# irfanfadhullah/unet_zoo

Measured on AMD Instinct MI355X. Metric: images/sec (fwd+bwd) at B=16 3x256x256, 1/2/4/8 MI355X, higher is better.
Workload: dtype bf16; 1 GPU; unet train step (zero_grad+fwd+BCE+bwd+clip+AdamW), B=16/GPU 3x256x256, random-init weights; global_batch=16, parallelism=dp1

## Files before the change

### include/unetzoo_hip.h

```cpp
#ifndef UNETZOO_HIP_H
#define UNETZOO_HIP_H

#include <stddef.h>
#include <stdint.h>

#ifdef __cplusplus
extern "C" {
#endif

#define UZ_ABI_VERSION 1

enum { UZ_F32 = 0, UZ_BF16 = 1 };

enum {
  UZ_OK = 0,
  UZ_EINVAL = -1,
  UZ_ENOTIMPL = -2
};

enum {
  UZ_TAPS_CONV = 0,
  UZ_TAPS_GATHER2X2 = 1,
  UZ_TAPS_CONV_UP2 = 2,
  UZ_TAPS_CONV_S2 = 3
// ... 4 lines not shown
};

int uz_abi_version(void);
const char* uz_last_error_string(void);
int uz_profile_arm(void* start_event, void* stop_event);
int uz_profile_disarm(void);
int uz_build_ablate(void);
const char* uz_source_hash(void);
int uz_clock_probe(int iters, void* out_pairs, int workgroups, void* stream);
int uz_set_cu_reserve(int n);
int uz_get_cu_reserve(void);

typedef struct uz_conv_desc {
  int dtype;
  int N, H, W;
  int Hin, Win;
  int Cin, ldx;
  int Nout, ldy;
  int ntaps, taps_mode, dil;
  int store_mode, Co;
  int Hout, Wout;
} uz_conv_desc;

int uz_conv_igemm_grid_m(const uz_conv_desc* d);
int uz_conv_igemm_kernel_name(const uz_conv_desc* d, int with_workspace, char* buf, int cap);
int uz_conv_igemm(const uz_conv_desc* d, const void* x, const void* w_packed, const float* bias,
                  void* y, float* stats_partial, void* stream);
int uz_conv_igemm_res(const uz_conv_desc* d, const void* x, const void* w_packed, const float* bias,
                      const void* res, int ldres, void* y, void* stream);
int uz_conv_igemm_res_ws(const uz_conv_desc* d, const void* x, const void* w_packed, const float* bias,
                         const void* res, int ldres, void* y, void* workspace, void* stream);
long long uz_conv_igemm_workspace_bytes(const uz_conv_desc* d);
int uz_conv_igemm_ws_grid_m(const uz_conv_desc* d);
int uz_conv_igemm_ws(const uz_conv_desc* d, const void* x, const void* w_packed, const float* bias,
                     void* y, float* stats_partial, void* workspace, void* stream);
int uz_conv_igemm_bnred_supported(const uz_conv_desc* d);
int uz_conv_igemm_bnred(const uz_conv_desc* d, const void* x, const void* w_packed, void* y, const void* bn_y,
                        int ld_bny, const float* scale, const float* shift, const float* mean, const float* invstd,
                        float* partial, void* stream);

int uz_conv_igemm_xf_supported(const uz_conv_desc* d);
int uz_conv_igemm_xf(const uz_conv_desc* d, const void* x, const float* in_scale, const float* in_shift,
                     const void* w_packed, const float* bias, void* y, float* stats_partial, void* stream);

int uz_conv_igemm_bnact_supported(const uz_conv_desc* d);
int uz_conv_igemm_bnact(const uz_conv_desc* d, const void* x, const void* w_packed, const float* bias,
                        const float* out_scale, const float* out_shift, int relu, void* y, void* stream);

typedef struct uz_wgrad_desc {
  int dtype;
  int N, H, W;
  int Hr, Wr;
  int Ci, ldl;
  int Cj, ldr;
  int ntaps, taps_mode, dil;
} uz_wgrad_desc;

int uz_wgrad_split(const uz_wgrad_desc* d);
long long uz_wgrad_workspace_bytes(const uz_wgrad_desc* d);
int uz_wgrad(const uz_wgrad_desc* d, const void* L, const void* R, float* out, void* workspace,
             void* stream);
int uz_wgrad_kernel_name(const uz_wgrad_desc* d, char* buf, int cap);
int uz_wgrad_xf_supported(const uz_wgrad_desc* d);
int uz_wgrad_xf(const uz_wgrad_desc* d, const void* L, const void* R, const float* r_scale, const float* r_shift,
                float* out, void* workspace, void* stream, int phase);
int uz_wgrad_phase(const uz_wgrad_desc* d, const void* L, const void* R, float* out, void* workspace, void* stream,
                   int phase);
typedef struct {
  uz_wgrad_desc desc;
  const void* L;
  const void* R;
  float* out;
} uz_wgrad_item;
long long uz_wgrad_multi_workspace_bytes(const uz_wgrad_item* items, int n);
int uz_wgrad_multi(const uz_wgrad_item* items, int n, void* workspace, void* stream);
long long uz_wgrad_batched_workspace_bytes(const uz_wgrad_desc* d, int batch);
int uz_wgrad_batched(const uz_wgrad_desc* d, int batch, const void* L, long long lb, const void* R, long long rb,
                     float* out, long long ob, void* workspace, void* stream);
int uz_wgrad_batched2(const uz_wgrad_desc* d, int batch, int batch2, const void* L, long long lb, long long lb2, const void* R,
                      long long rb, long long rb2, float* out, long long ob, void* workspace, void* stream);

int uz_conv3x3_first_supported(int dtype, int C, int Cout);
int uz_conv3x3_first_rows(int N, int H, int W);
int uz_conv3x3_first_fwd(int dtype, const float* x, int N, int C, int H, int W, const float* w, const float* bias, int Cout,
                         void* y, int ldy, float* stats, void* stream);
int uz_conv3x3_first_fwd_bnact(int dtype, const float* x, int N, int C, int H, int W, const float* w, const float* bias,
                               int Cout, const float* out_scale, const float* out_shift, int relu, void* y, int ldy,
                               void* stream);
long long uz_conv3x3_first_wgrad_workspace_bytes(int N, int H, int W, int Cout);
int uz_conv3x3_first_wgrad(int dtype, const float* x, int N, int C, int H, int W, const void* dy, int lddy, int Cout, float* dw,
                           void* workspace, void* stream);
int uz_conv3x3_first_wgrad_bn(int dtype, const float* x, int N, int C, int H, int W, const void* g, int ldg, const void* y,
                              int ldy, const float* scale, const float* shift, const float* mean, const float* invstd,
                              const double* sums, double count, int Cout, float* dw, void* workspace, void* stream);

enum { UZ_PACK_CONV_FWD = 0, UZ_PACK_CONV_DGRAD = 1, UZ_PACK_CONVT_FWD = 2, UZ_PACK_CONVT_DGRAD = 3,
       UZ_PACK_IM2COL = 4, UZ_PACK_VEC_REPEAT = 5 };
int uz_pack_weights(int dtype, int mode, const float* w, int Co, int Ci, int T, int Kpad, void* dst,
                    void* stream);
typedef struct uz_pack_item {
  const float* src;
  void* dst;
  long long begin;
  int mode, Co, Ci, T, Kpad;
  int pad_;
} uz_pack_item;
int uz_pack_weights_batched(int dtype, const uz_pack_item* items_device, int n_items,
                            long long total_elements, void* stream);
typedef struct uz_pack3x3_item {
  const float* src;
  void* dst_fwd;
  void* dst_dgrad;
  int Co, Ci;
  int tile_begin;
  int pad_;
} uz_pack3x3_item;
int uz_pack_conv3x3_batched(int dtype, const uz_pack3x3_item* items_device, int n_items, int total_tiles,
                            void* stream);

int uz_im2col3x3_nchw(int dtype, const float* x_nchw, int N, int C, int H, int W, int Kpad, void* dst,
                      void* stream);

int uz_bn_finalize(const float* stats_partial, int grid_m, int C, double count, const float* gamma,
                   const float* beta, float eps, float momentum, float* running_mean,
                   float* running_var, float* scale, float* shift, float* mean, float* invstd,
                   void* stream);
int uz_bn_eval_scale(int C, const float* gamma, const float* beta, const float* running_mean,
                     const float* running_var, float eps, float* scale, float* shift, void* stream);

int uz_bn_relu_apply(int dtype, const void* y, int ldy, const float* scale, const float* shift,
                     int N, int H, int W, int C, void* act, int lda, void* pooled, int ldp,
                     void* stream);
int uz_bn_relu_add_apply(int dtype, const void* y, int ldy, const float* scale, const float* shift,
                         int N, int H, int W, int C, const void* res, int ldr, void* act, int lda,
                         void* pooled, int ldp, int pool_ceil, void* stream);
int uz_bn_relu_add_apply_fin(int dtype, const void* y, int ldy, const float* stats_partial, int rows, double count,
                             const float* gamma, const float* beta, float eps, float momentum, float* running_mean,
                             float* running_var, float* vec, int* flag, int N, int H, int W, int C, const void* res, int ldr,
                             void* act, int lda, void* pooled, int ldp, int pool_ceil, void* stream);

typedef struct uz_bnbwd_desc {
  int dtype;
  int N, H, W, C;
  int ldy, ldg0, ldg1, ldgp, lddy;
  int pool_ceil;
} uz_bnbwd_desc;
int uz_colstats_rows(int dtype, int P, int C);
int uz_colstats(int dtype, const void* x, int ld, int P, int C, float* partial, void* stream);
long long uz_bn_relu_bwd_workspace_bytes(const uz_bnbwd_desc* d, int has_pool_grad);
int uz_bn_relu_bwd_reduce(const uz_bnbwd_desc* d, const void* y, const float* scale,
                          const float* shift, const float* mean, const float* invstd, const void* g0,
                          const void* g1, const void* gpool, void* workspace, double* sums,
                          float* dgamma, float* dbeta, void* stream);
int uz_bn_relu_bwd_apply(const uz_bnbwd_desc* d, const void* y, const float* scale,
                         const float* shift, const float* mean, const float* invstd, const void* g0,
                         const void* g1, const void* gpool, const double* sums, double count,
                         void* dy, void* stream);
int uz_bn_relu_bwd_reduce_rows(const uz_bnbwd_desc* d, const void* y, const float* scale, const float* shift,
                               const float* mean, const float* invstd, const void* g0, const void* g1, const void* gpool,
                               void* workspace, void* stream);
int uz_bn_relu_bwd_apply_fin(const uz_bnbwd_desc* d, const void* y, const float* scale, const float* shift,
                             const float* mean, const float* invstd, const void* g0, const void* g1, const void* gpool,
                             const float* partial, int rows, double* sums, float* dgamma, float* dbeta, int* flag,
                             double count, void* dy, void* stream);
int uz_bn_bwd_finalize(const float* partial, int rows, int C, double* sums, float* dgamma, float* dbeta, void* stream);
int uz_bn_relu_bwd_apply_head_supported(int dtype, int C, int Kout);
int uz_bn_relu_bwd_apply_head(const uz_bnbwd_desc* d, const void* y, const float* scale, const float* shift, const float* mean,
                              const float* invstd, const float* g_nchw, const float* w, int Kout, const double* sums,
                              double count, void* dy, void* stream);

int uz_outconv_fwd(int dtype, const void* x, int ldx, int N, int HW, int C, const float* w,
                   const float* b, int Kout, float* out_nchw, void* stream);
int uz_outconv_fwd_xf(int dtype, const void* y, int ldy, int N, int HW, int C, const float* scale, const float* shift,
                      const float* w, const float* b, int Kout, float* out_nchw, void* stream);
long long uz_outconv_bwd_workspace_bytes(int dtype, int N, int HW, int C, int Kout);
int uz_outconv_bwd(int dtype, const void* x, int ldx, int N, int HW, int C, const float* w, int Kout,
                   const float* g_nchw, void* dx, int lddx, float* dw, float* db, void* workspace,
                   void* stream);
int uz_outconv_bwd_rows(int dtype, int N, int HW, int C);
int uz_outconv_bwd_bnred(int dtype, const void* x, int ldx, int N, int HW, int C, const float* w, int Kout,
                         const float* g_nchw, void* dx, int lddx, float* dw, float* db, void* workspace,
                         const void* bn_y, int ld_bny, const float* scale, const float* shift, const float* mean,
                         const float* invstd, float* bn_partial, void* stream);

int uz_attn_grid(int dtype, int P, int channels);
int uz_attn_psi_fwd(int dtype, const void* g1raw, int ldg, const void* x1raw, int ldx, const float* vec_g,
                    const float* vec_x, const float* wpsi, const float* bpsi ,
                    int P, int F, float* q, float* partial , void* stream);
int uz_attn_gate_fwd(int dtype, const void* x, int ldx, const float* q, const float* vec_q, int P, int C,
                     void* out, int ldo, void* stream);
int uz_attn_bwd_psi(int dtype, const void* dout, int ldd, const void* x, int ldx, const float* q,
                    const float* vec_q, int P, int C, void* dx_direct, int lddx, float* dz,
                    float* partial , void* stream);
int uz_attn_bwd_reduce(int dtype, const void* g1raw, int ldg, const void* x1raw, int ldx, const float* q,
                       const float* dz, const float* wpsi, const float* vec_g, const float* vec_x,
                       const float* vec_q, const double* a01, int P, int F,
                       float* partial , void* stream);
int uz_attn_bwd_apply(int dtype, const void* g1raw, int ldg, const void* x1raw, int ldx, const float* q,
                      const float* dz, const float* wpsi, const float* vec_g, const float* vec_x,
                      const float* vec_q, const double* a01, const double* totals, int P, int F,
                      void* dg1raw, int lddg, void* dx1raw, int lddx, void* stream);
int uz_sum_rows(const float* partial, int rows, int n, double* out, void* stream);
int uz_sum_rows_f32(const float* partial, int rows, int n, float* out0, int n0, float* out1, void* stream);
int uz_sum_rows_f32_ld(const float* partial, int ld, int rows, int n, float* out0, int n0, float* out1,
                       void* stream);
int uz_sum2x2(int dtype, const void* du, int ldu, int N, int H, int W, int C, void* dx, int lddx,
              void* stream);

int uz_bilinear_fwd(int dtype, const void* x, int ldx, long long x_img_stride, int N, int Hi, int Wi,
                    int C, void* y, int ldy, long long y_img_stride, int Ho, int Wo, void* stream);
int uz_bilinear_bwd(int dtype, const void* g, int ldg, long long g_img_stride, int N, int Hi, int Wi,
                    int C, void* dx, int lddx, long long dx_img_stride, int Ho, int Wo, void* stream);
int uz_resize_bilinear_fwd(int dtype, const void* x, int ldx, long long x_img_stride, int N, int Hi, int Wi,
                           int C, void* y, int ldy, long long y_img_stride, int Ho, int Wo, int align_corners,
                           void* stream);
int uz_resize_bilinear_bwd(int dtype, const void* g, int ldg, long long g_img_stride, int N, int Hi, int Wi,
                           int C, void* dx, int lddx, long long dx_img_stride, int Ho, int Wo, int align_corners,
                           void* stream);
int uz_resample2(int dtype, const void* src, int lds, int N, int Hs, int Ws, int C, void* dst, int ldd, int Hd,
                 int Wd, int mode, void* stream);
int uz_pool_grad_combine(int dtype, int N, int H, int W, int C, const void* act, int lda, const void* g0,
                         int ldg0, const void* g1, int ldg1, const void* gp, int ldgp, void* out, int ldo,
                         int pool_ceil, void* stream);
int uz_sideconv3x3_fwd(int dtype, const void* x, int ldx, int N, int H, int W, int C, const float* w,
                       const float* bias, float* taps_ws, float* out, long long out_img_stride,
                       void* stream);
long long uz_sideconv3x3_bwd_workspace_bytes(int dtype, int N, int H, int W, int C);
int uz_sideconv3x3_bwd(int dtype, const void* x, int ldx, int N, int H, int W, int C, const float* w,
                       const float* g, long long g_img_stride, void* dx, int lddx, float* dw, float* db,
                       void* workspace, void* stream);
int uz_fuse1x1_fwd(const float* d, int N, int HW, int Cc, int K, const float* w, const float* b,
                   float* out, void* stream);
long long uz_fuse1x1_bwd_workspace_bytes(int N, int HW, int Cc, int K);
int uz_fuse1x1_bwd(const float* d, int N, int HW, int Cc, int K, const float* w, const float* g,
                   const float* const* g_extra, int n_extra, float* dcat, float* dw, float* db,
                   void* workspace, void* stream);

int uz_patchify(int dtype, const float* x_nchw, int N, int C, int H, int W, int patch, int Kpad,
                void* out, void* stream);

enum { UZ_LN_PLAIN = 0, UZ_LN_MERGE = 1, UZ_LN_EXPAND = 2 };
typedef struct uz_ln_desc {
  int dtype, N, Ho, Wo, C;
  int ldx, ldy, ldr, ldg, lddx;
  int mode, r;
  float eps;
  int act;
} uz_ln_desc;
int uz_layernorm_fwd(const uz_ln_desc* d, const void* x, const float* gamma, const float* beta,
                     const void* res, const float* image_scale, void* y, float* stats, void* stream);
int uz_layernorm_bwd_rows(const uz_ln_desc* d);
int uz_layernorm_bwd(const uz_ln_desc* d, const void* x, const float* gamma, const float* stats,
                     const void* g, const float* image_scale, void* dx, float* partial, void* stream);
int uz_layernorm_act_bwd(const uz_ln_desc* d, const void* x, const float* gamma, const float* beta,
                         const float* stats, const void* g, void* dx, float* partial, void* stream);
int uz_ln_head_fwd(const uz_ln_desc* d, const void* x, const float* gamma, const float* beta, const float* w,
                   const float* b , int K, float* logits, float* stats, void* stream);
long long uz_ln_head_bwd_workspace_bytes(const uz_ln_desc* d, int K);
int uz_ln_head_bwd(const uz_ln_desc* d, const void* x, const float* gamma, const float* beta, const float* w,
                   int K, const float* stats, const float* dlogits, void* dx, float* dgamma, float* dbeta,
                   float* dw, float* db , float* workspace, void* stream);

typedef struct uz_winattn_desc {
  int dtype, B, H, W, C, heads, ws, shift, Nt;
  int ldq, ldo;
  float scale;
} uz_winattn_desc;
int uz_winattn_fwd(const uz_winattn_desc* d, const void* qkv, const float* tau, const float* bias,
                   void* out, float* lse, void* stream);
int uz_cpb_fwd(const float* idx, const float* w1, const float* b1, const float* w2, const float* b2, int R,
               int hidden, int heads, float* bias, void* stream);
int uz_cpb_bwd(const float* idx, const float* w1, const float* b1, const float* w2, const float* G, int R,
               int hidden, int heads, float* dw1, float* db1, float* dw2, float* db2, void* stream);
typedef struct {
  const float* idx;
  const float* w1;
  const float* b1;
  const float* w2;
  const float* b2;
  int R, hidden, heads, reserved;
  float* bias;
  const float* G;
  float* dw1;
  float* db1;
  float* dw2;
  float* db2;
} uz_cpb_item;
int uz_cpb_fwd_batched(const uz_cpb_item* items, int n, void* stream);
long long uz_cpb_bwd_batched_workspace_bytes(const uz_cpb_item* items, int n);
int uz_cpb_bwd_batched(const uz_cpb_item* items, int n, float* workspace, void* stream);
int uz_winattn_bwd_rows(const uz_winattn_desc* d);
int uz_winattn_bwd(const uz_winattn_desc* d, const void* qkv, const float* tau, const float* bias,
                   const void* out, const float* lse, const void* dout, int lddo, void* dqkv, int lddq,
                   float* partial, void* stream);

int uz_colsum(int dtype, const void* x, int ld, int P, int C, float* out, void* stream);
long long uz_colsum_workspace_bytes(int dtype, int P, int C);
int uz_colsum_ws(int dtype, const void* x, int ld, int P, int C, float* out, void* workspace, void* stream);

long long uz_clip_adamw_workspace_bytes(void);
int uz_clip_adamw(float* p, const float* g, float* m, float* v, long long n, float lr, float beta1,
                  float beta2, float eps, float weight_decay, float max_norm, float* step, void* workspace,
                  void* stream);

int uz_gelu_fwd(int dtype, const void* x, int ldx, void* y, int ldy, long long P, int C, void* stream);
int uz_gelu_bwd(int dtype, const void* x, int ldx, const void* g, int ldg, void* dx, int lddx, long long P,
                int C, void* stream);
int uz_dwconv3x3(int dtype, const void* x, int ldx, const float* w_taps, const float* bias, void* y, int ldy,
                 int N, int H, int W, int C, int flags, void* stream);
int uz_dwconv3x3_wgrad_rows(int dtype, int N, int H, int W, int C);
int uz_dwconv3x3_wgrad(int dtype, const void* x, int ldx, const void* g, int ldg, float* part, int N, int H,
                       int W, int C, void* stream);
int uz_space_to_depth(int dtype, const void* src, int lds, void* dst, int ldd, int N, int Ho, int Wo, int C, int r,
                      int inverse, void* stream);
int uz_space_to_depth_crop(int dtype, const void* src, int lds, void* dst, int ldd, int N, int H, int W, int C, int r,
                           int inverse, void* stream);
int uz_im2col_nchw(int dtype, const float* x_nchw, int N, int C, int H, int W, int k, int stride, int pad, int Kpad,
                   void* out, void* stream);
typedef struct uz_sra_desc {
  int dtype, B, N, NK, heads, head_dim, kps;
  int ldq, ldk, ldv, ldo;
  float scale;
} uz_sra_desc;
int uz_sra_fwd(const uz_sra_desc* d, const void* q, const void* k, const void* v, void* out, float* lse,
               void* stream);
long long uz_sra_bwd_workspace_bytes(const uz_sra_desc* d);
int uz_sra_bwd(const uz_sra_desc* d, const void* q, const void* k, const void* v, const void* o, const float* lse,
               const void* go, int ldgo, void* dq, int lddq, void* dkv, int lddkv, void* workspace, void* stream);

long long uz_bce_dice_workspace_bytes(long long n);
int uz_bce_dice(const float* logits, const float* target, long long n, float* dlogits, float* out2, void* workspace,
                void* stream);

#define UZ_REGION_MAX_ITEMS 64
typedef struct uz_region_item {
  const float* logits;
  const float* target;
  float* dlogits;
  float weight;
} uz_region_item;
typedef struct uz_region_desc {
  int n_items;
  long long n;
  int groups;
  float w_bce, w_region, alpha, beta, smooth, gamma, pos_weight;
  int metric_item;
} uz_region_desc;
long long uz_region_loss_workspace_bytes(const uz_region_desc* d);
int uz_region_loss(const uz_region_desc* d, const uz_region_item* items, float* out2 , void* workspace,
                   void* stream);

#define UZ_CLASS_MAX_ITEMS 16
#define UZ_CLASS_MAX_K 32
#define UZ_CLASS_REDUCE_BATCH 0
#define UZ_CLASS_REDUCE_IMAGE 1
typedef struct uz_class_item {
  const float* logits;
  float* dlogits;
  float weight;
} uz_class_item;
typedef struct uz_class_desc {
  int n_items;
  int N, K;
  long long HW;
  float w_ce, w_dice, smooth, label_smoothing;
  int ignore_index;
  int reduce;
  int include_background;
  int square;
  int metric_item;
} uz_class_desc;
long long uz_class_loss_workspace_bytes(const uz_class_desc* d);
int uz_class_loss(const uz_class_desc* d, const uz_class_item* items, const int* labels,
                  const float* class_weight , float* out2 ,
                  long long* counts , void* workspace, void* stream);

typedef struct uz_colsum_item {
  const void* x;
  float* out;
  int P, C, ld, reserved;
} uz_colsum_item;
typedef struct uz_sum_rows_item {
  const float* partial;
  float* out0;
  float* out1;
  int rows, n, n0, reserved;
} uz_sum_rows_item;
int uz_sum_rows_f32_batched(const uz_sum_rows_item* items, int n, void* stream);
long long uz_colsum_batched_workspace_bytes(int dtype, const uz_colsum_item* items, int n);
int uz_colsum_batched(int dtype, const uz_colsum_item* items, int n, void* workspace, void* stream);

int uz_add_relu(int dtype, const void* a, int lda, const void* b, int ldb, void* out, int ldo, long long P, int C,
                void* stream);
int uz_relu_bwd(int dtype, const void* out, int ldo, const void* g, int ldg, void* dx, int lddx, long long P, int C,
                void* stream);

int uz_pil_resample_h_u8(const void* src, int H, int Win, int C, const int* bounds, const int* kk, int ksize, int Wout,
                         void* dst, void* stream);
int uz_pil_resample_v_f32(const void* src, int Hin, int W, int C, const int* bounds, const int* kk, int ksize, int Hout,
                          const float* mean_host, const float* std_host, int mode, float* out, void* stream);

typedef struct uz_gemm_desc {
  int dtype, batch, M, N, K;
  int ldx, ldw, ldy, ldres;
  long long xb, wb, yb, resb;
  int batch2;
  long long xb2, wb2, yb2, resb2;
} uz_gemm_desc;
int uz_gemm_nt(const uz_gemm_desc* d, const void* x, const void* w, const float* bias, const void* res, void* y,
               void* stream);
long long uz_softmax_workspace_bytes(int batch, int rows, int cols, int axis);
int uz_softmax_fwd(int dtype, void* s, int ld, long long sb, int batch, int rows, int cols, int axis, float scale,
                   void* workspace, void* stream);
int uz_softmax_bwd(int dtype, const void* a, void* g, int ld, long long sb, int batch, int rows, int cols, int axis,
                   float scale, float* dot, int dot_given, void* stream);
int uz_adaptive_avgpool_fwd(int dtype, const void* x, int ldx, int N, int Hi, int Wi, int C, void* y, int ldy, int Ho,
                            int Wo, void* stream);
int uz_adaptive_avgpool_bwd(int dtype, const void* g, int ldg, int N, int Hi, int Wi, int C, void* dx, int lddx, int Ho,
                            int Wo, int accumulate, void* stream);
int uz_rowdot_f32(int dtype, const float* a, int lda, const void* b, int ldb, long long rows, int C, float* out,
                  void* stream);
int uz_cast_rows(int dtype, const float* src, int lds, void* dst, int ldd, long long rows, int C, int accumulate,
                 void* stream);
int uz_add_map(int dtype, const void* x, int ldx, const float* map, void* out, int ldo, long long P, int HW, int C,
               void* stream);

int uz_dropout(int dtype, const void* x, int ldx, const float* u, float p, void* out, int ldo, long long P, int C,
               void* stream);

int uz_chanscale_relu(int dtype, int mode, const void* g, int ldg, const void* x, int ldx, const float* s, const float* a,
                      int N, int HW, int C, void* out, int ldo, void* stream);

int uz_chanattn_probs_fwd(int dtype, const float* scores, int B, int H, int C, int KV, float scale, float eps, void* pcat,
                          void* pcat_t, void* stream);
int uz_chanattn_probs_bwd(int dtype, const float* scores, const float* dpc, int B, int H, int C, int KV, float scale,
                          float eps, void* ds, void* ds_t, void* stream);

typedef struct uz_conv5x5_desc {
  int dtype;
  int N, H, W;
  int Cin, ldx;
  int Nout, ldy;
  int ksize;
} uz_conv5x5_desc;
int uz_conv5x5_grid_m(const uz_conv5x5_desc* d);
int uz_conv5x5(const uz_conv5x5_desc* d, const void* x, const void* w_packed, const float* bias, void* y, float* stats,
               void* stream);
typedef struct uz_wgrad5x5_desc {
  int dtype;
  int N, H, W;
  int Ci, ldl;
  int Cj, ldr;
  int ksize;
  int CiOut, CjOut;
} uz_wgrad5x5_desc;
long long uz_wgrad5x5_workspace_bytes(const uz_wgrad5x5_desc* d);
int uz_wgrad5x5(const uz_wgrad5x5_desc* d, const void* L, const void* R, float* out, void* workspace, void* stream);

int uz_bn_elu_apply(int dtype, const void* x, int ldx, const float* scale, const float* shift, int N, int HW, int C,
                    const void* res, int ldres, void* out, int ldo, void* out2, int ldo2, const float* mask2, int flags,
                    void* stream);
typedef struct uz_bn_elu_bwd_desc {
  int dtype;
  int N, HW, C;
  int ldx, ldo, ldg0, ldg1, ldg2, lddx, ldgres;
  int flags;
} uz_bn_elu_bwd_desc;
int uz_bn_elu_bwd_rows(const uz_bn_elu_bwd_desc* d);
int uz_bn_elu_bwd_reduce(const uz_bn_elu_bwd_desc* d, const void* x, const void* out, const void* g0, const void* g1,
                         const void* g2, const float* mask2, const float* scale, const float* shift, const float* mean,
                         const float* invstd, float* partials, void* stream);
int uz_bn_elu_bwd_apply(const uz_bn_elu_bwd_desc* d, const void* x, const void* out, const void* g0, const void* g1,
                        const void* g2, const float* mask2, const float* scale, const float* shift, const float* mean,
                        const float* invstd, const double* sums, void* dx, void* gres, void* stream);

#define UZ_AUGMENT_MASK_NONE 0
#define UZ_AUGMENT_MASK_F32 1
#define UZ_AUGMENT_MASK_I32 2
typedef struct uz_augment_desc {
  int N, C, H, W;
  int mask_kind;
  int Cm;
  int G;
  float p_hflip, p_vflip, rotate, scale_min, scale_max, translate, brightness, contrast;
  float image_fill, mask_fill;
  int label_fill;
} uz_augment_desc;
int uz_augment_params(const uz_augment_desc* d, const float* u, float* params, void* stream);
int uz_augment_grid(const uz_augment_desc* d, int* units );
int uz_augment_apply(const uz_augment_desc* d, const float* image, const void* mask, const float* params, const float* disp,
                     float* image_out, void* mask_out, void* stream);

#define UZ_PATCH_IMAGE_F32 0
#define UZ_PATCH_IMAGE_U8 1
#define UZ_PATCH_MASK_NONE 0
#define UZ_PATCH_MASK_F32 1
#define UZ_PATCH_MASK_I32 2
typedef struct uz_patch_desc {
  int M, C, H, W;
  int image_kind;
  int mask_kind;
  int Cm;
  int P;
  int B, h, w;
  int use_indices;
  float pos;
  float jitter;
} uz_patch_desc;
long long uz_patch_index_bytes(const uz_patch_desc* d);
int uz_patch_index(const uz_patch_desc* d, const void* mask, int* index, void* stream);
int uz_patch_draw(const uz_patch_desc* d, const float* u, const int* indices , const int* index, const void* mask,
                  int* coords, void* stream);
int uz_patch_cut_grid(const uz_patch_desc* d, int* units );
int uz_patch_cut(const uz_patch_desc* d, const void* image, const void* mask, const int* coords, const float* norm ,
                 float* image_out, void* mask_out, void* stream);

#define UZ_SURFACE_BINARY 0
#define UZ_SURFACE_CLASS 1
typedef struct uz_surface_desc {
  int mode;
  int N, C, H, W;
  int first_class;
  int ignore_index;
  int reserved;
  double q;
  double spacing;
} uz_surface_desc;
long long uz_surface_workspace_bytes(const uz_surface_desc* d);
int uz_surface_grid(const uz_surface_desc* d, int* units );
int uz_surface_metrics(const uz_surface_desc* d, const float* logits, const void* target, float* out, long long* stats,
                       void* workspace, void* stream);

#define UZ_BOUNDARY_BINARY 0
#define UZ_BOUNDARY_CLASS 1
typedef struct uz_boundary_item {
  const float* logits;
  float* dlogits;
  float weight;
} uz_boundary_item;
typedef struct uz_boundary_desc {
  int mode;
  int n_items;
  int N, C, H, W;
  int first_class;
  int ignore_index;
  int metric_item;
  float spacing;
} uz_boundary_desc;
long long uz_boundary_workspace_bytes(const uz_boundary_desc* d);
int uz_boundary_grid(const uz_boundary_desc* d, int* units );
int uz_boundary_loss(const uz_boundary_desc* d, const uz_boundary_item* items, const void* target,
                     const float* scales , const float* base_loss ,
                     float* out , int* sd2 , void* workspace, void* stream);

#define UZ_LOVASZ_BINARY 0
#define UZ_LOVASZ_CLASS 1
#define UZ_LOVASZ_PRESENT 0
#define UZ_LOVASZ_ALL 1
typedef struct uz_lovasz_item {
  const float* logits;
  float* dlogits;
  float weight;
} uz_lovasz_item;
typedef struct uz_lovasz_desc {
  int mode;
  int n_items;
  int N, C, H, W;
  int per_image;
  int classes;
  int ignore_index;
  int main_item;
} uz_lovasz_desc;
long long uz_lovasz_workspace_bytes(const uz_lovasz_desc* d);
int uz_lovasz_grid(const uz_lovasz_desc* d, int* units );
int uz_lovasz_loss(const uz_lovasz_desc* d, const uz_lovasz_item* items, const void* target,
                   const float* scales , const float* base_loss ,
                   float* out , float* errors , int* ranks ,
                   void* workspace, void* stream);

#define UZ_POST_BINARY 0
#define UZ_POST_CLASS 1
#define UZ_POST_MAX_KEEP 8
typedef struct uz_postproc_desc {
  int mode;
  int N, C, H, W;
  int first_class;
  int connectivity;
  int fill_holes;
  int min_area;
  int keep_largest;
  float thr;
  int reserved;
} uz_postproc_desc;
long long uz_postproc_workspace_bytes(const uz_postproc_desc* d);
int uz_postproc_grid(const uz_postproc_desc* d, int* units );
int uz_postproc(const uz_postproc_desc* d, const float* x, unsigned char* mask, int* labels ,
                unsigned char* class_map , long long* stats, long long* comps, void* workspace, void* stream);

typedef struct uz_tta_desc {
  int mode;
  int N, C, H, W;
  int views;
  int dtype;
  int reserved;
} uz_tta_desc;
int uz_tta_num_views(int views);
// ... 32 lines not shown
```

### unet_zoo_amd/_lib.py

```python
from __future__ import annotations

import ctypes
import os
from ctypes import POINTER, Structure, c_char_p, c_double, c_float, c_int, c_void_p

import torch

UZ_F32, UZ_BF16 = 0, 1
TAPS_CONV, TAPS_GATHER2X2, TAPS_CONV_UP2, TAPS_CONV_S2 = 0, 1, 2, 3
STORE_PLAIN, STORE_SHUFFLE2X2 = 0, 1
PACK_CONV_FWD, PACK_CONV_DGRAD, PACK_CONVT_FWD, PACK_CONVT_DGRAD, PACK_IM2COL, PACK_VEC_REPEAT = range(6)

LIB_NAME = "libunetzoo_hip.so"
LIB_PATH = os.environ.get("UNET_ZOO_AMD_LIB") or os.path.join(os.path.dirname(os.path.abspath(__file__)), LIB_NAME)

EXPORTS = (
    "uz_abi_version", "uz_last_error_string", "uz_build_ablate", "uz_source_hash", "uz_set_cu_reserve", "uz_get_cu_reserve", "uz_clock_probe", "uz_conv_igemm_grid_m", "uz_conv_igemm",
    "uz_wgrad_split", "uz_wgrad_workspace_bytes", "uz_wgrad", "uz_wgrad_kernel_name", "uz_wgrad_phase", "uz_wgrad_xf_supported", "uz_wgrad_xf", "uz_conv3x3_first_supported", "uz_conv3x3_first_rows", "uz_conv3x3_first_fwd",
    "uz_conv3x3_first_wgrad_workspace_bytes", "uz_conv3x3_first_wgrad", "uz_conv3x3_first_wgrad_bn", "uz_pack_weights", "uz_pack_weights_batched", "uz_pack_conv3x3_batched", "uz_im2col3x3_nchw", "uz_bn_finalize",
    "uz_bn_eval_scale", "uz_bn_relu_apply", "uz_bn_relu_bwd_workspace_bytes", "uz_bn_relu_bwd_reduce", "uz_bn_relu_bwd_apply",
    "uz_outconv_fwd", "uz_outconv_fwd_xf", "uz_outconv_bwd_workspace_bytes", "uz_outconv_bwd", "uz_outconv_bwd_rows", "uz_outconv_bwd_bnred", "uz_bn_relu_bwd_apply_head_supported", "uz_bn_relu_bwd_apply_head",
    "uz_colsum",
    "uz_attn_grid", "uz_attn_psi_fwd", "uz_attn_gate_fwd", "uz_attn_bwd_psi", "uz_attn_bwd_reduce",
    "uz_attn_bwd_apply", "uz_sum_rows", "uz_sum_rows_f32", "uz_sum2x2",
    "uz_bn_relu_add_apply", "uz_bn_relu_add_apply_fin", "uz_bn_relu_bwd_reduce_rows", "uz_bn_relu_bwd_apply_fin", "uz_bilinear_fwd", "uz_bilinear_bwd", "uz_resize_bilinear_fwd", "uz_resize_bilinear_bwd", "uz_resample2",
    "uz_pool_grad_combine",
    "uz_sideconv3x3_fwd", "uz_sideconv3x3_bwd_workspace_bytes", "uz_sideconv3x3_bwd",
    "uz_fuse1x1_fwd", "uz_fuse1x1_bwd_workspace_bytes", "uz_fuse1x1_bwd",
    "uz_conv_igemm_workspace_bytes", "uz_conv_igemm_ws_grid_m", "uz_conv_igemm_ws",
    "uz_conv_igemm_bnred_supported", "uz_conv_igemm_bnred", "uz_conv_igemm_xf_supported", "uz_conv_igemm_xf", "uz_conv_igemm_kernel_name", "uz_bn_bwd_finalize", "uz_profile_arm", "uz_profile_disarm",
    "uz_patchify", "uz_layernorm_fwd", "uz_layernorm_bwd_rows", "uz_layernorm_bwd", "uz_layernorm_act_bwd",
    "uz_ln_head_fwd", "uz_ln_head_bwd_workspace_bytes", "uz_ln_head_bwd", "uz_sum_rows_f32_ld",
    "uz_winattn_fwd", "uz_winattn_bwd_rows", "uz_winattn_bwd",
    "uz_colsum_workspace_bytes", "uz_colsum_ws", "uz_colstats_rows", "uz_colstats", "uz_cpb_fwd", "uz_cpb_bwd",
    "uz_cpb_fwd_batched", "uz_cpb_bwd_batched_workspace_bytes", "uz_cpb_bwd_batched",
    "uz_clip_adamw_workspace_bytes", "uz_clip_adamw",
    "uz_gelu_fwd", "uz_gelu_bwd", "uz_dwconv3x3", "uz_dwconv3x3_wgrad_rows", "uz_dwconv3x3_wgrad",
    "uz_space_to_depth", "uz_space_to_depth_crop", "uz_im2col_nchw", "uz_sra_fwd", "uz_sra_bwd_workspace_bytes", "uz_sra_bwd",
    "uz_bce_dice_workspace_bytes", "uz_bce_dice", "uz_colsum_batched_workspace_bytes", "uz_colsum_batched", "uz_sum_rows_f32_batched", "uz_conv_igemm_res", "uz_wgrad_multi_workspace_bytes", "uz_wgrad_multi", "uz_conv_igemm_res_ws",
    "uz_add_relu", "uz_relu_bwd", "uz_pil_resample_h_u8", "uz_pil_resample_v_f32",
    "uz_gemm_nt", "uz_softmax_fwd", "uz_softmax_bwd", "uz_adaptive_avgpool_fwd", "uz_adaptive_avgpool_bwd",
    "uz_rowdot_f32", "uz_cast_rows", "uz_wgrad_batched_workspace_bytes", "uz_wgrad_batched", "uz_wgrad_batched2",
    "uz_softmax_workspace_bytes", "uz_add_map", "uz_dropout", "uz_chanscale_relu", "uz_chanattn_probs_fwd", "uz_chanattn_probs_bwd",
    "uz_conv5x5_grid_m", "uz_conv5x5", "uz_wgrad5x5_workspace_bytes", "uz_wgrad5x5",
    "uz_bn_elu_apply", "uz_bn_elu_bwd_rows", "uz_bn_elu_bwd_reduce", "uz_bn_elu_bwd_apply",
    "uz_conv_igemm_bnact_supported", "uz_conv_igemm_bnact", "uz_conv3x3_first_fwd_bnact",
    "uz_region_loss_workspace_bytes", "uz_region_loss",
    "uz_class_loss_workspace_bytes", "uz_class_loss",
    "uz_augment_params", "uz_augment_grid", "uz_augment_apply",
    "uz_patch_index_bytes", "uz_patch_index", "uz_patch_draw", "uz_patch_cut_grid", "uz_patch_cut",
    "uz_surface_workspace_bytes", "uz_surface_grid", "uz_surface_metrics",
    "uz_boundary_workspace_bytes", "uz_boundary_grid", "uz_boundary_loss",
    "uz_lovasz_workspace_bytes", "uz_lovasz_grid", "uz_lovasz_loss",
    "uz_postproc_workspace_bytes", "uz_postproc_grid", "uz_postproc",
    "uz_tta_num_views", "uz_flip_views", "uz_tta_merge", "uz_mask_decide",
    "uz_tile_plan", "uz_tile_gather", "uz_tile_blend",
)


class ConvDesc(Structure):
    _fields_ = [(n, c_int) for n in (
        "dtype", "N", "H", "W", "Hin", "Win", "Cin", "ldx", "Nout", "ldy", "ntaps", "taps_mode",
        "dil", "store_mode", "Co", "Hout", "Wout")]


class WgradDesc(Structure):
    _fields_ = [(n, c_int) for n in (
        "dtype", "N", "H", "W", "Hr", "Wr", "Ci", "ldl", "Cj", "ldr", "ntaps", "taps_mode", "dil")]


class Conv5Desc(Structure):
    _fields_ = [(n, c_int) for n in ("dtype", "N", "H", "W", "Cin", "ldx", "Nout", "ldy", "ksize")]


class Wgrad5Desc(Structure):
    _fields_ = [(n, c_int) for n in ("dtype", "N", "H", "W", "Ci", "ldl", "Cj", "ldr", "ksize", "CiOut", "CjOut")]


class BnEluBwdDesc(Structure):
    _fields_ = [(n, c_int) for n in ("dtype", "N", "HW", "C", "ldx", "ldo", "ldg0", "ldg1", "ldg2", "lddx", "ldgres", "flags")]


class BnBwdDesc(Structure):
    _fields_ = [(n, c_int) for n in (
        "dtype", "N", "H", "W", "C", "ldy", "ldg0", "ldg1", "ldgp", "lddy", "pool_ceil")]


class LnDesc(Structure):
    _fields_ = [(n, c_int) for n in ("dtype", "N", "Ho", "Wo", "C", "ldx", "ldy", "ldr", "ldg", "lddx", "mode", "r")] \
        + [("eps", c_float), ("act", c_int)]


class WinAttnDesc(Structure):
    _fields_ = [(n, c_int) for n in ("dtype", "B", "H", "W", "C", "heads", "ws", "shift", "Nt", "ldq", "ldo")] \
        + [("scale", c_float)]


class SraDesc(Structure):
    _fields_ = [(n, c_int) for n in ("dtype", "B", "N", "NK", "heads", "head_dim", "kps", "ldq", "ldk", "ldv", "ldo")] \
        + [("scale", c_float)]


class GemmDesc(Structure):
    _fields_ = [(n, c_int) for n in ("dtype", "batch", "M", "N", "K", "ldx", "ldw", "ldy", "ldres")] \
        + [(n, ctypes.c_longlong) for n in ("xb", "wb", "yb", "resb")] + [("batch2", c_int)] \
        + [(n, ctypes.c_longlong) for n in ("xb2", "wb2", "yb2", "resb2")]


class WgradItem(Structure):
    _fields_ = [("desc", WgradDesc), ("L", c_void_p), ("R", c_void_p), ("out", c_void_p)]


class SumRowsItem(Structure):
    _fields_ = [("partial", c_void_p), ("out0", c_void_p), ("out1", c_void_p), ("rows", c_int), ("n", c_int), ("n0", c_int),
                ("reserved", c_int)]


class ColsumItem(Structure):
    _fields_ = [("x", c_void_p), ("out", c_void_p), ("P", c_int), ("C", c_int), ("ld", c_int), ("reserved", c_int)]


LN_PLAIN, LN_MERGE, LN_EXPAND = 0, 1, 2


class CpbItem(Structure):
    _fields_ = [(n, c_void_p) for n in ("idx", "w1", "b1", "w2", "b2")] \
        + [(n, c_int) for n in ("R", "hidden", "heads", "reserved")] \
        + [(n, c_void_p) for n in ("bias", "G", "dw1", "db1", "dw2", "db2")]


class PackItem(Structure):
    _fields_ = [("src", c_void_p), ("dst", c_void_p), ("begin", ctypes.c_longlong), ("mode", c_int),
                ("Co", c_int), ("Ci", c_int), ("T", c_int), ("Kpad", c_int), ("pad_", c_int)]


class Pack3x3Item(Structure):
    _fields_ = [("src", c_void_p), ("dst_fwd", c_void_p), ("dst_dgrad", c_void_p), ("Co", c_int), ("Ci", c_int),
                ("tile_begin", c_int), ("pad_", c_int)]


REGION_MAX_ITEMS = 64


class RegionItem(Structure):
    _fields_ = [("logits", c_void_p), ("target", c_void_p), ("dlogits", c_void_p), ("weight", c_float)]


class RegionDesc(Structure):
    _fields_ = [("n_items", c_int), ("n", ctypes.c_longlong), ("groups", c_int)] \
        + [(n, c_float) for n in ("w_bce", "w_region", "alpha", "beta", "smooth", "gamma", "pos_weight")] \
        + [("metric_item", c_int)]


CLASS_MAX_ITEMS = 16
CLASS_MAX_K = 32
CLASS_REDUCE_BATCH, CLASS_REDUCE_IMAGE = 0, 1


class ClassItem(Structure):
    _fields_ = [("logits", c_void_p), ("dlogits", c_void_p), ("weight", c_float)]


class ClassDesc(Structure):
    _fields_ = [("n_items", c_int), ("N", c_int), ("K", c_int), ("HW", ctypes.c_longlong)] \
        + [(n, c_float) for n in ("w_ce", "w_dice", "smooth", "label_smoothing")] \
        + [(n, c_int) for n in ("ignore_index", "reduce", "include_background", "square", "metric_item")]


AUGMENT_MASK_NONE, AUGMENT_MASK_F32, AUGMENT_MASK_I32 = 0, 1, 2


class AugmentDesc(Structure):
    _fields_ = [(n, c_int) for n in ("N", "C", "H", "W", "mask_kind", "Cm", "G")] \
        + [(n, c_float) for n in ("p_hflip", "p_vflip", "rotate", "scale_min", "scale_max", "translate", "brightness",
                                  "contrast", "image_fill", "mask_fill")] \
        + [("label_fill", c_int)]


PATCH_IMAGE_F32, PATCH_IMAGE_U8 = 0, 1
PATCH_MASK_NONE, PATCH_MASK_F32, PATCH_MASK_I32 = 0, 1, 2


class PatchDesc(Structure):
    _fields_ = [(n, c_int) for n in ("M", "C", "H", "W", "image_kind", "mask_kind", "Cm", "P", "B", "h", "w", "use_indices")] \
        + [("pos", c_float), ("jitter", c_float)]


SURFACE_BINARY, SURFACE_CLASS = 0, 1
SURFACE_MAX_HW = 4096


class SurfaceDesc(Structure):
    _fields_ = [(n, c_int) for n in ("mode", "N", "C", "H", "W", "first_class", "ignore_index", "reserved")] \
        + [("q", c_double), ("spacing", c_double)]


BOUNDARY_BINARY, BOUNDARY_CLASS = 0, 1
BOUNDARY_MAX_HW = 4096


class BoundaryItem(Structure):
    _fields_ = [("logits", c_void_p), ("dlogits", c_void_p), ("weight", c_float)]


class BoundaryDesc(Structure):
    _fields_ = [(n, c_int) for n in ("mode", "n_items", "N", "C", "H", "W", "first_class", "ignore_index", "metric_item")] \
        + [("spacing", c_float)]


LOVASZ_BINARY, LOVASZ_CLASS = 0, 1
LOVASZ_PRESENT, LOVASZ_ALL = 0, 1
LOVASZ_MAX_SEGMENT = 1 << 22
LOVASZ_MAX_ELEMENTS = 1 << 28


class LovaszItem(Structure):
    _fields_ = [("logits", c_void_p), ("dlogits", c_void_p), ("weight", c_float)]


class LovaszDesc(Structure):
    _fields_ = [(n, c_int) for n in ("mode", "n_items", "N", "C", "H", "W", "per_image", "classes", "ignore_index", "main_item")]


POST_BINARY, POST_CLASS = 0, 1
POST_MAX_KEEP = 8
POST_MAX_HW = 4096
TTA_VIEWS = {"identity": 1, "hflip": 2, "vflip": 4, "hvflip": 8}


class PostprocDesc(Structure):
    _fields_ = [(n, c_int) for n in ("mode", "N", "C", "H", "W", "first_class", "connectivity", "fill_holes", "min_area",
                                     "keep_largest")] + [("thr", c_float), ("reserved", c_int)]


class TtaDesc(Structure):
    _fields_ = [(n, c_int) for n in ("mode", "N", "C", "H", "W", "views", "dtype", "reserved")]


TILE_MAX_AXIS, TILE_MAX_COVER = 256, 8
TILE_PADS = {"constant": 0, "reflect": 1}


class TileGatherDesc(Structure):
    _fields_ = [(n, c_int) for n in ("N", "C", "H", "W", "th", "tw", "ny", "nx", "pad_mode", "t0", "tn", "reserved")]


class TileBlendDesc(Structure):
    _fields_ = [(n, c_int) for n in ("N", "C", "H", "W", "th", "tw", "ny", "nx")]


class HipLibraryError(RuntimeError):
    pass


_lib = None


def load():
    global _lib
    if _lib is not None:
        return _lib
    if not os.path.exists(LIB_PATH):
        raise HipLibraryError(
            f"{LIB_PATH} not found: the HIP kernel library is not built. Run "
            "`python -c 'import __graft_entry__ as g; g.build()'` from the repo root. "
            "unet_zoo_amd has no CPU fallback.")
    lib = ctypes.CDLL(LIB_PATH)
    lib.uz_abi_version.restype = c_int
    lib.uz_last_error_string.restype = c_char_p
    lib.uz_source_hash.restype = c_char_p
    lib.uz_source_hash.argtypes = []
    vp, ip, fp = c_void_p, c_int, c_float
    lib.uz_set_cu_reserve.argtypes = [c_int]
    lib.uz_clock_probe.argtypes = [c_int, vp, c_int, vp]
    lib.uz_get_cu_reserve.argtypes = []
    lib.uz_conv_igemm_grid_m.argtypes = [POINTER(ConvDesc)]
    lib.uz_conv_igemm.argtypes = [POINTER(ConvDesc), vp, vp, vp, vp, vp, vp]
    lib.uz_conv_igemm_res.argtypes = [POINTER(ConvDesc), vp, vp, vp, vp, ip, vp, vp]
    lib.uz_conv_igemm_res_ws.argtypes = [POINTER(ConvDesc), vp, vp, vp, vp, ip, vp, vp, vp]
    lib.uz_conv_igemm_workspace_bytes.argtypes = [POINTER(ConvDesc)]
    lib.uz_conv_igemm_ws_grid_m.argtypes = [POINTER(ConvDesc)]
    lib.uz_conv_igemm_ws.argtypes = [POINTER(ConvDesc), vp, vp, vp, vp, vp, vp, vp]
    lib.uz_conv_igemm_bnred_supported.argtypes = [POINTER(ConvDesc)]
    lib.uz_conv_igemm_xf_supported.argtypes = [POINTER(ConvDesc)]
    lib.uz_conv_igemm_xf.argtypes = [POINTER(ConvDesc), vp, vp, vp, vp, vp, vp, vp, vp]
    lib.uz_conv_igemm_bnact_supported.argtypes = [POINTER(ConvDesc)]
    lib.uz_conv_igemm_bnact.argtypes = [POINTER(ConvDesc), vp, vp, vp, vp, vp, c_int, vp, vp]
    lib.uz_conv_igemm_kernel_name.argtypes = [POINTER(ConvDesc), c_int, c_char_p, c_int]
    lib.uz_profile_arm.argtypes = [vp, vp]
    lib.uz_profile_disarm.argtypes = []
    lib.uz_conv_igemm_bnred.argtypes = [POINTER(ConvDesc), vp, vp, vp, vp, c_int, vp, vp, vp, vp, vp, vp]
    lib.uz_bn_bwd_finalize.argtypes = [vp, c_int, c_int, vp, vp, vp, vp]
    lib.uz_patchify.argtypes = [ip, vp, ip, ip, ip, ip, ip, ip, vp, vp]
    lib.uz_layernorm_fwd.argtypes = [POINTER(LnDesc), vp, vp, vp, vp, vp, vp, vp, vp]
    lib.uz_layernorm_act_bwd.argtypes = [POINTER(LnDesc), vp, vp, vp, vp, vp, vp, vp, vp]
    lib.uz_layernorm_bwd_rows.argtypes = [POINTER(LnDesc)]
    lib.uz_layernorm_bwd.argtypes = [POINTER(LnDesc), vp, vp, vp, vp, vp, vp, vp, vp]
    lib.uz_ln_head_fwd.argtypes = [POINTER(LnDesc), vp, vp, vp, vp, vp, ip, vp, vp, vp]
    lib.uz_ln_head_bwd_workspace_bytes.argtypes = [POINTER(LnDesc), ip]
    lib.uz_ln_head_bwd.argtypes = [POINTER(LnDesc), vp, vp, vp, vp, ip, vp, vp, vp, vp, vp, vp, vp, vp, vp]
    lib.uz_sum_rows_f32_ld.argtypes = [vp, ip, ip, ip, vp, ip, vp, vp]
    lib.uz_winattn_fwd.argtypes = [POINTER(WinAttnDesc), vp, vp, vp, vp, vp, vp]
    lib.uz_winattn_bwd_rows.argtypes = [POINTER(WinAttnDesc)]
    lib.uz_winattn_bwd.argtypes = [POINTER(WinAttnDesc), vp, vp, vp, vp, vp, vp, ip, vp, ip, vp, vp]
    lib.uz_colstats_rows.argtypes = [ip, ip, ip]
    lib.uz_colstats.argtypes = [ip, vp, ip, ip, ip, vp, vp]
    lib.uz_cpb_fwd.argtypes = [vp, vp, vp, vp, vp, ip, ip, ip, vp, vp]
    lib.uz_cpb_bwd.argtypes = [vp, vp, vp, vp, vp, ip, ip, ip, vp, vp, vp, vp, vp]
    lib.uz_cpb_fwd_batched.argtypes = [vp, ip, vp]
    lib.uz_cpb_bwd_batched_workspace_bytes.argtypes = [vp, ip]
    lib.uz_cpb_bwd_batched.argtypes = [vp, ip, vp, vp]
    lib.uz_clip_adamw_workspace_bytes.argtypes = []
    lib.uz_clip_adamw.argtypes = [vp, vp, vp, vp, ctypes.c_longlong, fp, fp, fp, fp, fp, fp, vp, vp, vp]
    lib.uz_wgrad_split.argtypes = [POINTER(WgradDesc)]
    lib.uz_wgrad_workspace_bytes.argtypes = [POINTER(WgradDesc)]
    lib.uz_wgrad.argtypes = [POINTER(WgradDesc), vp, vp, vp, vp, vp]
    lib.uz_wgrad_kernel_name.argtypes = [POINTER(WgradDesc), c_char_p, c_int]
    lib.uz_wgrad_phase.argtypes = [POINTER(WgradDesc), vp, vp, vp, vp, vp, c_int]
    lib.uz_wgrad_xf_supported.argtypes = [POINTER(WgradDesc)]
    lib.uz_wgrad_xf.argtypes = [POINTER(WgradDesc), vp, vp, vp, vp, vp, vp, vp, c_int]
    lib.uz_conv3x3_first_supported.argtypes = [ip, ip, ip]
    lib.uz_conv3x3_first_rows.argtypes = [ip, ip, ip]
    lib.uz_conv3x3_first_fwd.argtypes = [ip, vp, ip, ip, ip, ip, vp, vp, ip, vp, ip, vp, vp]
    lib.uz_conv3x3_first_fwd_bnact.argtypes = [ip, vp, ip, ip, ip, ip, vp, vp, ip, vp, vp, ip, vp, ip, vp]
    lib.uz_conv3x3_first_wgrad_workspace_bytes.argtypes = [ip, ip, ip, ip]
    lib.uz_conv3x3_first_wgrad_workspace_bytes.restype = ctypes.c_longlong
    lib.uz_conv3x3_first_wgrad.argtypes = [ip, vp, ip, ip, ip, ip, vp, ip, ip, vp, vp, vp]
    lib.uz_conv3x3_first_wgrad_bn.argtypes = [ip, vp, ip, ip, ip, ip, vp, ip, vp, ip, vp, vp, vp, vp, vp, ctypes.c_double, ip, vp, vp, vp]
    lib.uz_pack_weights.argtypes = [ip, ip, vp, ip, ip, ip, ip, vp, vp]
    lib.uz_pack_weights_batched.argtypes = [ip, vp, ip, ctypes.c_longlong, vp]
    lib.uz_pack_conv3x3_batched.argtypes = [ip, vp, ip, ip, vp]
    lib.uz_im2col3x3_nchw.argtypes = [ip, vp, ip, ip, ip, ip, ip, vp, vp]
    lib.uz_bn_finalize.argtypes = [vp, ip, ip, c_double, vp, vp, fp, fp, vp, vp, vp, vp, vp, vp, vp]
    lib.uz_bn_eval_scale.argtypes = [ip, vp, vp, vp, vp, fp, vp, vp, vp]
    lib.uz_bn_relu_apply.argtypes = [ip, vp, ip, vp, vp, ip, ip, ip, ip, vp, ip, vp, ip, vp]
    lib.uz_bn_relu_bwd_workspace_bytes.argtypes = [POINTER(BnBwdDesc), ip]
    lib.uz_bn_relu_bwd_reduce.argtypes = [POINTER(BnBwdDesc), vp, vp, vp, vp, vp, vp, vp, vp, vp, vp,
                                          vp, vp, vp]
    lib.uz_bn_relu_bwd_apply.argtypes = [POINTER(BnBwdDesc), vp, vp, vp, vp, vp, vp, vp, vp, vp,
                                         c_double, vp, vp]
    lib.uz_outconv_fwd.argtypes = [ip, vp, ip, ip, ip, ip, vp, vp, ip, vp, vp]
    lib.uz_outconv_fwd_xf.argtypes = [ip, vp, ip, ip, ip, ip, vp, vp, vp, vp, ip, vp, vp]
    lib.uz_outconv_bwd_workspace_bytes.argtypes = [ip, ip, ip, ip, ip]
    lib.uz_outconv_bwd.argtypes = [ip, vp, ip, ip, ip, ip, vp, ip, vp, vp, ip, vp, vp, vp, vp]
    lib.uz_outconv_bwd_rows.argtypes = [ip, ip, ip, ip]
    lib.uz_bn_relu_bwd_apply_head_supported.argtypes = [ip, ip, ip]
    lib.uz_bn_relu_bwd_apply_head.argtypes = [POINTER(BnBwdDesc), vp, vp, vp, vp, vp, vp, vp, ip, vp, ctypes.c_double, vp, vp]
    lib.uz_outconv_bwd_bnred.argtypes = [ip, vp, ip, ip, ip, ip, vp, ip, vp, vp, ip, vp, vp, vp, vp, ip, vp, vp, vp, vp, vp, vp]
    lib.uz_colsum.argtypes = [ip, vp, ip, ip, ip, vp, vp]
    lib.uz_colsum_workspace_bytes.argtypes = [ip, ip, ip]
    lib.uz_colsum_ws.argtypes = [ip, vp, ip, ip, ip, vp, vp, vp]
    lib.uz_attn_grid.argtypes = [ip, ip, ip]
    lib.uz_attn_psi_fwd.argtypes = [ip, vp, ip, vp, ip, vp, vp, vp, vp, ip, ip, vp, vp, vp]
    lib.uz_attn_gate_fwd.argtypes = [ip, vp, ip, vp, vp, ip, ip, vp, ip, vp]
    lib.uz_attn_bwd_psi.argtypes = [ip, vp, ip, vp, ip, vp, vp, ip, ip, vp, ip, vp, vp, vp]
    lib.uz_attn_bwd_reduce.argtypes = [ip, vp, ip, vp, ip, vp, vp, vp, vp, vp, vp, vp, ip, ip, vp, vp]
    lib.uz_attn_bwd_apply.argtypes = [ip, vp, ip, vp, ip, vp, vp, vp, vp, vp, vp, vp, vp, ip, ip, vp, ip,
                                      vp, ip, vp]
    lib.uz_sum_rows.argtypes = [vp, ip, ip, vp, vp]
    lib.uz_sum_rows_f32.argtypes = [vp, ip, ip, vp, ip, vp, vp]
    lib.uz_sum2x2.argtypes = [ip, vp, ip, ip, ip, ip, ip, vp, ip, vp]
    ll = ctypes.c_longlong
    lib.uz_bn_relu_add_apply.argtypes = [ip, vp, ip, vp, vp, ip, ip, ip, ip, vp, ip, vp, ip, vp, ip, ip, vp]
    lib.uz_bn_relu_add_apply_fin.argtypes = [ip, vp, ip, vp, ip, ctypes.c_double, vp, vp, c_float, c_float, vp, vp, vp, vp,
                                             ip, ip, ip, ip, vp, ip, vp, ip, vp, ip, ip, vp]
    lib.uz_bn_relu_bwd_reduce_rows.argtypes = [POINTER(BnBwdDesc), vp, vp, vp, vp, vp, vp, vp, vp, vp, vp]
    lib.uz_bn_relu_bwd_apply_fin.argtypes = [POINTER(BnBwdDesc), vp, vp, vp, vp, vp, vp, vp, vp, vp, ip, vp, vp, vp, vp,
                                             ctypes.c_double, vp, vp]
    lib.uz_bilinear_fwd.argtypes = [ip, vp, ip, ll, ip, ip, ip, ip, vp, ip, ll, ip, ip, vp]
    lib.uz_bilinear_bwd.argtypes = [ip, vp, ip, ll, ip, ip, ip, ip, vp, ip, ll, ip, ip, vp]
    lib.uz_resize_bilinear_fwd.argtypes = [ip, vp, ip, ll, ip, ip, ip, ip, vp, ip, ll, ip, ip, ip, vp]
    lib.uz_resize_bilinear_bwd.argtypes = [ip, vp, ip, ll, ip, ip, ip, ip, vp, ip, ll, ip, ip, ip, vp]
    lib.uz_resample2.argtypes = [ip, vp, ip, ip, ip, ip, ip, vp, ip, ip, ip, ip, vp]
    lib.uz_pool_grad_combine.argtypes = [ip, ip, ip, ip, ip, vp, ip, vp, ip, vp, ip, vp, ip, vp, ip, ip, vp]
    lib.uz_sideconv3x3_fwd.argtypes = [ip, vp, ip, ip, ip, ip, ip, vp, vp, vp, vp, ll, vp]
    lib.uz_sideconv3x3_bwd_workspace_bytes.argtypes = [ip, ip, ip, ip, ip]
    lib.uz_sideconv3x3_bwd.argtypes = [ip, vp, ip, ip, ip, ip, ip, vp, vp, ll, vp, ip, vp, vp, vp, vp]
    lib.uz_fuse1x1_fwd.argtypes = [vp, ip, ip, ip, ip, vp, vp, vp, vp]
    lib.uz_fuse1x1_bwd_workspace_bytes.argtypes = [ip, ip, ip, ip]
    lib.uz_fuse1x1_bwd.argtypes = [vp, ip, ip, ip, ip, vp, vp, POINTER(c_void_p), ip, vp, vp, vp, vp, vp]
    lib.uz_sum_rows_f32_batched.argtypes = [POINTER(SumRowsItem), ip, vp]
    lib.uz_wgrad_multi_workspace_bytes.argtypes = [POINTER(WgradItem), ip]
    lib.uz_wgrad_multi_workspace_bytes.restype = ctypes.c_longlong
    lib.uz_wgrad_multi.argtypes = [POINTER(WgradItem), ip, vp, vp]
    lib.uz_colsum_batched_workspace_bytes.argtypes = [ip, POINTER(ColsumItem), ip]
    lib.uz_colsum_batched.argtypes = [ip, POINTER(ColsumItem), ip, vp, vp]
    lib.uz_bce_dice_workspace_bytes.argtypes = [ll]
    lib.uz_bce_dice.argtypes = [vp, vp, ll, vp, vp, vp, vp]
    lib.uz_gelu_fwd.argtypes = [ip, vp, ip, vp, ip, ll, ip, vp]
    lib.uz_gelu_bwd.argtypes = [ip, vp, ip, vp, ip, vp, ip, ll, ip, vp]
    lib.uz_dwconv3x3.argtypes = [ip, vp, ip, vp, vp, vp, ip, ip, ip, ip, ip, ip, vp]
    lib.uz_dwconv3x3_wgrad_rows.argtypes = [ip, ip, ip, ip, ip]
    lib.uz_dwconv3x3_wgrad.argtypes = [ip, vp, ip, vp, ip, vp, ip, ip, ip, ip, vp]
    lib.uz_space_to_depth.argtypes = [ip, vp, ip, vp, ip, ip, ip, ip, ip, ip, ip, vp]
    lib.uz_space_to_depth_crop.argtypes = [ip, vp, ip, vp, ip, ip, ip, ip, ip, ip, ip, vp]
    lib.uz_im2col_nchw.argtypes = [ip, vp, ip, ip, ip, ip, ip, ip, ip, ip, vp, vp]
    lib.uz_sra_fwd.argtypes = [POINTER(SraDesc), vp, vp, vp, vp, vp, vp]
    lib.uz_sra_bwd_workspace_bytes.argtypes = [POINTER(SraDesc)]
    lib.uz_sra_bwd.argtypes = [POINTER(SraDesc), vp, vp, vp, vp, vp, vp, ip, vp, ip, vp, ip, vp, vp]
    lib.uz_add_relu.argtypes = [ip, vp, ip, vp, ip, vp, ip, ll, ip, vp]
    lib.uz_relu_bwd.argtypes = [ip, vp, ip, vp, ip, vp, ip, ll, ip, vp]
    lib.uz_pil_resample_h_u8.argtypes = [vp, ip, ip, ip, vp, vp, ip, ip, vp, vp]
    lib.uz_pil_resample_v_f32.argtypes = [vp, ip, ip, ip, vp, vp, ip, ip, POINTER(c_float), POINTER(c_float), ip, vp, vp]
    lib.uz_wgrad_batched_workspace_bytes.argtypes = [POINTER(WgradDesc), ip]
    lib.uz_wgrad_batched.argtypes = [POINTER(WgradDesc), ip, vp, ll, vp, ll, vp, ll, vp, vp]
    lib.uz_wgrad_batched2.argtypes = [POINTER(WgradDesc), ip, ip, vp, ll, ll, vp, ll, ll, vp, ll, vp, vp]
    lib.uz_gemm_nt.argtypes = [POINTER(GemmDesc), vp, vp, vp, vp, vp, vp]
    lib.uz_softmax_workspace_bytes.argtypes = [ip, ip, ip, ip]
    lib.uz_softmax_fwd.argtypes = [ip, vp, ip, ll, ip, ip, ip, ip, c_float, vp, vp]
    lib.uz_chanattn_probs_fwd.argtypes = [ip, vp, ip, ip, ip, ip, c_float, c_float, vp, vp, vp]
    lib.uz_chanattn_probs_bwd.argtypes = [ip, vp, vp, ip, ip, ip, ip, c_float, c_float, vp, vp, vp]
    lib.uz_dropout.argtypes = [ip, vp, ip, vp, c_float, vp, ip, ll, ip, vp]
    lib.uz_chanscale_relu.argtypes = [ip, ip, vp, ip, vp, ip, vp, vp, ip, ip, ip, vp, ip, vp]
    lib.uz_add_map.argtypes = [ip, vp, ip, vp, vp, ip, ll, ip, ip, vp]
    lib.uz_softmax_bwd.argtypes = [ip, vp, vp, ip, ll, ip, ip, ip, ip, c_float, vp, ip, vp]
    lib.uz_adaptive_avgpool_fwd.argtypes = [ip, vp, ip, ip, ip, ip, ip, vp, ip, ip, ip, vp]
    lib.uz_adaptive_avgpool_bwd.argtypes = [ip, vp, ip, ip, ip, ip, ip, vp, ip, ip, ip, ip, vp]
    lib.uz_rowdot_f32.argtypes = [ip, vp, ip, vp, ip, ll, ip, vp, vp]
    lib.uz_cast_rows.argtypes = [ip, vp, ip, vp, ip, ll, ip, ip, vp]
    lib.uz_conv5x5_grid_m.argtypes = [POINTER(Conv5Desc)]
    lib.uz_conv5x5.argtypes = [POINTER(Conv5Desc), vp, vp, vp, vp, vp, vp]
    lib.uz_wgrad5x5_workspace_bytes.argtypes = [POINTER(Wgrad5Desc)]
    lib.uz_wgrad5x5.argtypes = [POINTER(Wgrad5Desc), vp, vp, vp, vp, vp]
    lib.uz_bn_elu_apply.argtypes = [ip, vp, ip, vp, vp, ip, ip, ip, vp, ip, vp, ip, vp, ip, vp, ip, vp]
    lib.uz_bn_elu_bwd_rows.argtypes = [POINTER(BnEluBwdDesc)]
    lib.uz_bn_elu_bwd_reduce.argtypes = [POINTER(BnEluBwdDesc), vp, vp, vp, vp, vp, vp, vp, vp, vp, vp, vp, vp]
    lib.uz_bn_elu_bwd_apply.argtypes = [POINTER(BnEluBwdDesc), vp, vp, vp, vp, vp, vp, vp, vp, vp, vp, vp, vp, vp, vp]
    lib.uz_region_loss_workspace_bytes.argtypes = [POINTER(RegionDesc)]
    lib.uz_region_loss.argtypes = [POINTER(RegionDesc), POINTER(RegionItem), vp, vp, vp]
    lib.uz_class_loss_workspace_bytes.argtypes = [POINTER(ClassDesc)]
    lib.uz_class_loss.argtypes = [POINTER(ClassDesc), POINTER(ClassItem), vp, vp, vp, vp, vp, vp]
    lib.uz_augment_params.argtypes = [POINTER(AugmentDesc), vp, vp, vp]
    lib.uz_augment_grid.argtypes = [POINTER(AugmentDesc), POINTER(c_int)]
    lib.uz_augment_apply.argtypes = [POINTER(AugmentDesc), vp, vp, vp, vp, vp, vp, vp]
    lib.uz_patch_index_bytes.argtypes = [POINTER(PatchDesc)]
    lib.uz_patch_index.argtypes = [POINTER(PatchDesc), vp, vp, vp]
    lib.uz_patch_draw.argtypes = [POINTER(PatchDesc), vp, vp, vp, vp, vp, vp]
    lib.uz_patch_cut_grid.argtypes = [POINTER(PatchDesc), POINTER(c_int)]
    lib.uz_patch_cut.argtypes = [POINTER(PatchDesc), vp, vp, vp, vp, vp, vp, vp]
    lib.uz_surface_workspace_bytes.argtypes = [POINTER(SurfaceDesc)]
    lib.uz_surface_grid.argtypes = [POINTER(SurfaceDesc), POINTER(c_int)]
    lib.uz_surface_metrics.argtypes = [POINTER(SurfaceDesc), vp, vp, vp, vp, vp, vp]
    lib.uz_boundary_workspace_bytes.argtypes = [POINTER(BoundaryDesc)]
    lib.uz_boundary_grid.argtypes = [POINTER(BoundaryDesc), POINTER(c_int)]
    lib.uz_boundary_loss.argtypes = [POINTER(BoundaryDesc), POINTER(BoundaryItem), vp, vp, vp, vp, vp, vp, vp]
    lib.uz_lovasz_workspace_bytes.argtypes = [POINTER(LovaszDesc)]
    lib.uz_lovasz_grid.argtypes = [POINTER(LovaszDesc), POINTER(c_int)]
    lib.uz_lovasz_loss.argtypes = [POINTER(LovaszDesc), POINTER(LovaszItem), vp, vp, vp, vp, vp, vp, vp, vp]
    lib.uz_postproc_workspace_bytes.argtypes = [POINTER(PostprocDesc)]
    lib.uz_postproc_grid.argtypes = [POINTER(PostprocDesc), POINTER(c_int)]
    lib.uz_postproc.argtypes = [POINTER(PostprocDesc), vp, vp, vp, vp, vp, vp, vp, vp]
    lib.uz_tta_num_views.argtypes = [c_int]
    lib.uz_flip_views.argtypes = [POINTER(TtaDesc), vp, POINTER(c_void_p), vp]
    lib.uz_tta_merge.argtypes = [POINTER(TtaDesc), POINTER(c_void_p), vp, vp]
    lib.uz_mask_decide.argtypes = [POINTER(TtaDesc), vp, c_float, c_int, vp, vp, vp]
    lib.uz_tile_plan.argtypes = [c_int, c_int, c_double, POINTER(c_int), c_int]
    lib.uz_tile_gather.argtypes = [POINTER(TileGatherDesc), POINTER(c_int), POINTER(c_int), vp, vp, vp]
    lib.uz_tile_blend.argtypes = [POINTER(TileBlendDesc), POINTER(c_int), POINTER(c_int), vp, vp, vp, vp, vp]
    for name in EXPORTS:
        fn = getattr(lib, name)
        if name not in ("uz_last_error_string", "uz_source_hash"):
            fn.restype = ctypes.c_longlong if name.endswith(("_workspace_bytes", "_index_bytes")) else c_int
    if lib.uz_abi_version() != 1:
        raise HipLibraryError("libunetzoo_hip.so ABI version mismatch; rebuild it")
    _lib = lib
    return lib


def _fail(rc: int, what: str):
    msg = load().uz_last_error_string().decode("utf-8", "replace")
    raise HipLibraryError(f"{what} failed (code {rc}): {msg}")


def check(rc: int, what: str) -> None:
    if rc != 0:
        _fail(rc, what)


def check_count(rc: int, what: str) -> int:
    if rc < 0:
        _fail(rc, what)
    return rc


def region_loss_workspace_bytes(desc: "RegionDesc") -> int:
    return check_count(load().uz_region_loss_workspace_bytes(ctypes.byref(desc)), "uz_region_loss_workspace_bytes")


def region_loss(desc: "RegionDesc", items, out2: torch.Tensor, workspace: torch.Tensor) -> None:
    check(load().uz_region_loss(ctypes.byref(desc), items, out2.data_ptr(), workspace.data_ptr(), stream_ptr()),
          "uz_region_loss")


def class_loss_workspace_bytes(desc: "ClassDesc") -> int:
    return check_count(load().uz_class_loss_workspace_bytes(ctypes.byref(desc)), "uz_class_loss_workspace_bytes")


def class_loss(desc: "ClassDesc", items, labels: torch.Tensor, class_weight, out2: torch.Tensor, counts: torch.Tensor,
               workspace: torch.Tensor) -> None:
    check(load().uz_class_loss(ctypes.byref(desc), items, labels.data_ptr(),
                               class_weight.data_ptr() if class_weight is not None else None, out2.data_ptr(),
                               counts.data_ptr() if counts is not None else None, workspace.data_ptr(), stream_ptr()),
          "uz_class_loss")


def surface_workspace_bytes(desc: "SurfaceDesc") -> int:
    return check_count(load().uz_surface_workspace_bytes(ctypes.byref(desc)), "uz_surface_workspace_bytes")


def surface_grid(desc: "SurfaceDesc") -> tuple:
    units = c_int(0)
    grid = check_count(load().uz_surface_grid(ctypes.byref(desc), ctypes.byref(units)), "uz_surface_grid")
    return grid, units.value


def surface_metrics(desc: "SurfaceDesc", logits: torch.Tensor, target: torch.Tensor, out: torch.Tensor, stats: torch.Tensor,
                    workspace: torch.Tensor) -> None:
    check(load().uz_surface_metrics(ctypes.byref(desc), logits.data_ptr(), target.data_ptr(), out.data_ptr(), stats.data_ptr(),
                                    workspace.data_ptr(), stream_ptr()), "uz_surface_metrics")


def boundary_workspace_bytes(desc: "BoundaryDesc") -> int:
    return check_count(load().uz_boundary_workspace_bytes(ctypes.byref(desc)), "uz_boundary_workspace_bytes")


def boundary_grid(desc: "BoundaryDesc") -> tuple:
    units = c_int(0)
    grid = check_count(load().uz_boundary_grid(ctypes.byref(desc), ctypes.byref(units)), "uz_boundary_grid")
    return grid, units.value


def boundary_loss(desc: "BoundaryDesc", items, target: torch.Tensor, scales: torch.Tensor, base_loss: torch.Tensor,
                  out2: torch.Tensor, sd2: torch.Tensor, workspace: torch.Tensor) -> None:
    check(load().uz_boundary_loss(ctypes.byref(desc), items, target.data_ptr(), scales.data_ptr(), base_loss.data_ptr(),
                                  out2.data_ptr(), sd2.data_ptr(), workspace.data_ptr(), stream_ptr()), "uz_boundary_loss")


def lovasz_workspace_bytes(desc: "LovaszDesc") -> int:
    return check_count(load().uz_lovasz_workspace_bytes(ctypes.byref(desc)), "uz_lovasz_workspace_bytes")


def lovasz_grid(desc: "LovaszDesc") -> tuple:
    units = c_int(0)
    grid = check_count(load().uz_lovasz_grid(ctypes.byref(desc), ctypes.byref(units)), "uz_lovasz_grid")
    return grid, units.value


def lovasz_loss(desc: "LovaszDesc", items, target: torch.Tensor, scales: torch.Tensor, base_loss: torch.Tensor,
                out2: torch.Tensor, errors: torch.Tensor, ranks: torch.Tensor, workspace: torch.Tensor) -> None:
    check(load().uz_lovasz_loss(ctypes.byref(desc), items, target.data_ptr(), scales.data_ptr(), base_loss.data_ptr(),
                                out2.data_ptr(), errors.data_ptr(), ranks.data_ptr(), workspace.data_ptr(), stream_ptr()),
          "uz_lovasz_loss")


def postproc_workspace_bytes(desc: "PostprocDesc") -> int:
    return check_count(load().uz_postproc_workspace_bytes(ctypes.byref(desc)), "uz_postproc_workspace_bytes")


def postproc_grid(desc: "PostprocDesc") -> tuple:
    units = c_int(0)
    grid = check_count(load().uz_postproc_grid(ctypes.byref(desc), ctypes.byref(units)), "uz_postproc_grid")
    return grid, units.value


def _ptr(t) -> "int | None":
    return t.data_ptr() if t is not None else None


def postproc(desc: "PostprocDesc", x: torch.Tensor, mask: torch.Tensor, labels, class_map, stats: torch.Tensor, comps: torch.Tensor,
             workspace: torch.Tensor) -> None:
    check(load().uz_postproc(ctypes.byref(desc), x.data_ptr(), mask.data_ptr(), _ptr(labels), _ptr(class_map), stats.data_ptr(),
                             comps.data_ptr(), workspace.data_ptr(), stream_ptr()), "uz_postproc")


def _ptr_table(tensors):
    return (c_void_p * len(tensors))(*[t.data_ptr() for t in tensors])


def flip_views(desc: "TtaDesc", x: torch.Tensor, views) -> None:
    check(load().uz_flip_views(ctypes.byref(desc), x.data_ptr(), _ptr_table(views), stream_ptr()), "uz_flip_views")


def tta_merge(desc: "TtaDesc", logits, prob: torch.Tensor) -> None:
    check(load().uz_tta_merge(ctypes.byref(desc), _ptr_table(logits), prob.data_ptr(), stream_ptr()), "uz_tta_merge")


def mask_decide(desc: "TtaDesc", x: torch.Tensor, thr: float, first_class: int, mask: torch.Tensor, class_map) -> None:
    check(load().uz_mask_decide(ctypes.byref(desc), x.data_ptr(), float(thr), int(first_class), mask.data_ptr(), _ptr(class_map),
                                stream_ptr()), "uz_mask_decide")


def tile_plan(size: int, window: int, overlap: float) -> list:
    starts = (c_int * TILE_MAX_AXIS)()
    n = check_count(load().uz_tile_plan(int(size), int(window), float(overlap), starts, TILE_MAX_AXIS), "uz_tile_plan")
    return [int(starts[i]) for i in range(n)]


def _int_table(values):
    return (c_int * len(values))(*[int(v) for v in values])


def tile_gather(desc: "TileGatherDesc", ys, xs, x: torch.Tensor, out: torch.Tensor) -> None:
    check(load().uz_tile_gather(ctypes.byref(desc), _int_table(ys), _int_table(xs), x.data_ptr(), out.data_ptr(), stream_ptr()),
          "uz_tile_gather")


def tile_blend(desc: "TileBlendDesc", ys, xs, tiles: torch.Tensor, gh: torch.Tensor, gw: torch.Tensor, out: torch.Tensor) -> None:
    check(load().uz_tile_blend(ctypes.byref(desc), _int_table(ys), _int_table(xs), tiles.data_ptr(), gh.data_ptr(), gw.data_ptr(),
                               out.data_ptr(), stream_ptr()), "uz_tile_blend")


def set_cu_reserve(n: int) -> None:
    check(load().uz_set_cu_reserve(int(n)), "uz_set_cu_reserve")


def get_cu_reserve() -> int:
# ... 46 lines not shown
```

### unet_zoo_amd/csrc/uz_eltwise.hip

```cpp
#include "uz_common.h"

namespace {

template <typename T> __device__ __forceinline__ void load_f(const T* p, float* f) {
  const Vec16<T> v = ld16(p);
#pragma unroll
  for (int i = 0; i < ElemTraits<T>::VEC; ++i) f[i] = (float)v.v[i];
}
template <typename T> __device__ __forceinline__ void store_f(T* p, const float* f) {
  Vec16<T> v;
#pragma unroll
  for (int i = 0; i < ElemTraits<T>::VEC; ++i) v.v[i] = (T)f[i];
  st16(p, v);
}

template <int EW>
__global__ __launch_bounds__(1024) void bn_finalize_kernel(
    const float* __restrict__ part, int grid_m, int C, double count, const float* __restrict__ gamma,
    const float* __restrict__ beta, float eps, float momentum, float* running_mean,
    float* running_var, float* scale, float* shift, float* mean, float* invstd) {
  constexpr int NG = 1024 / EW;
  __shared__ double sh[2][NG][EW + 1];
  const int cl = threadIdx.x % EW, g = threadIdx.x / EW;
  const int c = blockIdx.x * EW + cl;
// ... 1503 lines not shown
  const int rc = bnbwd_check(d, g0, g1, gpool);
  if (rc != UZ_OK) return rc;
  UZ_REQUIRE(y && scale && shift && mean && invstd && sums && dy, "uz_bn_relu_bwd_apply: null pointer");
  UZ_REQUIRE(count > 0, "uz_bn_relu_bwd_apply: count");
  const int vec = d->dtype == UZ_BF16 ? 8 : 4;
  UZ_REQUIRE(d->lddy % vec == 0 && d->lddy >= d->C, "uz_bn_relu_bwd_apply: bad lddy");
  BnBwdArgs a = bnbwd_args(d, y, scale, shift, mean, invstd, g0, g1, gpool);
  a.sums = const_cast<double*>(sums);
  a.dy = dy;
  a.inv_count = 1.0 / count;
  hipStream_t s = (hipStream_t)stream;
  return d->dtype == UZ_BF16 ? bnbwd_launch<bf16_t, 2>(d, a, gpool != nullptr, s)
                             : bnbwd_launch<float, 2>(d, a, gpool != nullptr, s);
}

extern "C" int uz_bn_relu_bwd_reduce_rows(const uz_bnbwd_desc* d, const void* y, const float* scale, const float* shift,
                                          const float* mean, const float* invstd, const void* g0, const void* g1,
                                          const void* gpool, void* workspace, void* stream) {
  const int rc = bnbwd_check(d, g0, g1, gpool);
  if (rc != UZ_OK) return rc;
  UZ_REQUIRE(y && scale && shift && mean && invstd && workspace, "uz_bn_relu_bwd_reduce_rows: null pointer");
  BnBwdArgs a = bnbwd_args(d, y, scale, shift, mean, invstd, g0, g1, gpool);
  a.partials = static_cast<float*>(workspace);
  hipStream_t s = (hipStream_t)stream;
  return d->dtype == UZ_BF16 ? bnbwd_launch<bf16_t, 1>(d, a, gpool != nullptr, s) : bnbwd_launch<float, 1>(d, a, gpool != nullptr, s);
}

extern "C" int uz_bn_relu_bwd_apply_fin(const uz_bnbwd_desc* d, const void* y, const float* scale, const float* shift,
                                        const float* mean, const float* invstd, const void* g0, const void* g1,
                                        const void* gpool, const float* partial, int rows, double* sums, float* dgamma,
                                        float* dbeta, int* flag, double count, void* dy, void* stream) {
  const int rc = bnbwd_check(d, g0, g1, gpool);
  if (rc != UZ_OK) return rc;
  UZ_REQUIRE(y && scale && shift && mean && invstd && sums && dy && partial && flag, "uz_bn_relu_bwd_apply_fin: null pointer");
  UZ_REQUIRE(count > 0 && rows > 0, "uz_bn_relu_bwd_apply_fin: count / rows");
  UZ_REQUIRE((dgamma == nullptr) == (dbeta == nullptr), "uz_bn_relu_bwd_apply_fin: dgamma/dbeta");
  const int vec = d->dtype == UZ_BF16 ? 8 : 4;
  UZ_REQUIRE(d->lddy % vec == 0 && d->lddy >= d->C, "uz_bn_relu_bwd_apply_fin: bad lddy");
  BnBwdArgs a = bnbwd_args(d, y, scale, shift, mean, invstd, g0, g1, gpool);
  a.sums = sums;
  a.dy = dy;
  a.inv_count = 1.0 / count;
  a.fin.part = partial; a.fin.rows = rows; a.fin.ew = fin_ew(rows, d->C);
  a.fin.sums = sums; a.fin.dgamma = dgamma; a.fin.dbeta = dbeta; a.fin.flag = flag;
  hipStream_t s = (hipStream_t)stream;
  dim3 grid, block;
  bnbwd_shape(d, gpool != nullptr, &grid, &block, 2);
  if ((long long)grid.x * grid.y < (d->C + a.fin.ew - 1) / a.fin.ew) {
    bnbwd_finalize(partial, rows, d->C, sums, dgamma, dbeta, s);
    UZ_LAUNCH_CHECK("uz_bn_relu_bwd_apply_fin(finalize)");
    a.fin = BnFin{};
    return d->dtype == UZ_BF16 ? bnbwd_launch<bf16_t, 2>(d, a, gpool != nullptr, s) : bnbwd_launch<float, 2>(d, a, gpool != nullptr, s);
  }
  return d->dtype == UZ_BF16 ? bnbwd_launch<bf16_t, 2, true>(d, a, gpool != nullptr, s)
                             : bnbwd_launch<float, 2, true>(d, a, gpool != nullptr, s);
}

extern "C" int uz_bn_relu_bwd_apply_head_supported(int dtype, int C, int Kout) {
  return dtype == UZ_BF16 && C > 0 && C % 8 == 0 && Kout >= 1 && Kout <= OUTCONV_MAXK;
}

extern "C" int uz_bn_relu_bwd_apply_head(const uz_bnbwd_desc* d, const void* y, const float* scale, const float* shift,
                                         const float* mean, const float* invstd, const float* g_nchw, const float* w,
                                         int Kout, const double* sums, double count, void* dy, void* stream) {
  UZ_REQUIRE(d != nullptr, "uz_bn_relu_bwd_apply_head: null descriptor");
  UZ_REQUIRE(uz_bn_relu_bwd_apply_head_supported(d->dtype, d->C, Kout), "uz_bn_relu_bwd_apply_head: dtype=%d C=%d Kout=%d unsupported",
             d->dtype, d->C, Kout);
  UZ_REQUIRE(y && scale && shift && mean && invstd && g_nchw && w && sums && dy, "uz_bn_relu_bwd_apply_head: null pointer");
  UZ_REQUIRE(d->N > 0 && d->H > 0 && d->W > 0 && (long long)d->N * d->H * d->W < (1LL << 31), "uz_bn_relu_bwd_apply_head: bad shape");
  UZ_REQUIRE(d->ldy % 8 == 0 && d->ldy >= d->C && d->lddy % 8 == 0 && d->lddy >= d->C, "uz_bn_relu_bwd_apply_head: bad ldy / lddy");
  UZ_REQUIRE((d->pool_ceil & 3) == 0, "uz_bn_relu_bwd_apply_head: a ReLU block without a pool only");
  UZ_REQUIRE(count > 0, "uz_bn_relu_bwd_apply_head: count");
  BnBwdHeadArgs a;
  a.y = static_cast<const bf16_t*>(y);
  a.dy = static_cast<bf16_t*>(dy);
  a.scale = scale;
  a.shift = shift;
  a.mean = mean;
  a.invstd = invstd;
  a.sums = sums;
  a.g = g_nchw;
  a.w = w;
  a.inv_count = 1.0 / count;
  a.P = d->N * d->H * d->W;
  a.HW = d->H * d->W;
  a.C = d->C;
  a.ldy = d->ldy;
  a.lddy = d->lddy;
  a.rev = (d->pool_ceil & 4) != 0;
  dim3 grid, block;
  bnbwd_shape(d, false, &grid, &block, 2);
  hipStream_t s = (hipStream_t)stream;
  UZ_KOUT_SWITCH(Kout, hipLaunchKernelGGL((bn_relu_bwd_head_kernel<KOUT>), grid, block, 0, s, a))
  UZ_LAUNCH_CHECK("uz_bn_relu_bwd_apply_head");
  return UZ_OK;
}

extern "C" int uz_outconv_fwd(int dtype, const void* x, int ldx, int N, int HW, int C, const float* w,
                              const float* b, int Kout, float* out_nchw, void* stream) {
  UZ_REQUIRE(dtype == UZ_F32 || dtype == UZ_BF16, "uz_outconv_fwd: bad dtype");
  const int vec = dtype == UZ_BF16 ? 8 : 4;
  UZ_REQUIRE(x && w && b && out_nchw, "uz_outconv_fwd: null pointer");
  UZ_REQUIRE(Kout >= 1 && Kout <= OUTCONV_MAXK, "uz_outconv_fwd: Kout=%d (max %d)", Kout, OUTCONV_MAXK);
  UZ_REQUIRE(C % vec == 0 && C / vec <= 64, "uz_outconv_fwd: C=%d unsupported", C);
  UZ_REQUIRE(ldx % vec == 0 && ldx >= C && N > 0 && HW > 0 && (long long)N * HW < (1LL << 31),
             "uz_outconv_fwd: bad shape");
  const int ppb = 256 / lanes_per_pixel(C / vec);
  const int grid = grid_for(((long long)N * HW + ppb - 1) / ppb, 1);
  hipStream_t s = (hipStream_t)stream;
  if (dtype == UZ_BF16) {
    UZ_KOUT_SWITCH(Kout, hipLaunchKernelGGL((outconv_fwd_kernel<bf16_t, KOUT>), dim3(grid), dim3(256), 0, s, (const bf16_t*)x, ldx, N, HW, C, w, b, out_nchw, (const float*)nullptr, (const float*)nullptr))
  } else {
    UZ_KOUT_SWITCH(Kout, hipLaunchKernelGGL((outconv_fwd_kernel<float, KOUT>), dim3(grid), dim3(256), 0, s, (const float*)x, ldx, N, HW, C, w, b, out_nchw, (const float*)nullptr, (const float*)nullptr))
  }
  UZ_LAUNCH_CHECK("uz_outconv_fwd");
  return UZ_OK;
}

extern "C" int uz_outconv_fwd_xf(int dtype, const void* y, int ldy, int N, int HW, int C, const float* scale,
                                 const float* shift, const float* w, const float* b, int Kout, float* out_nchw,
                                 void* stream) {
  UZ_REQUIRE(dtype == UZ_BF16, "uz_outconv_fwd_xf: bf16 only");
  UZ_REQUIRE(y && scale && shift && w && b && out_nchw, "uz_outconv_fwd_xf: null pointer");
  UZ_REQUIRE(Kout >= 1 && Kout <= OUTCONV_MAXK, "uz_outconv_fwd_xf: Kout=%d (max %d)", Kout, OUTCONV_MAXK);
  UZ_REQUIRE(C % 8 == 0 && C / 8 <= 64, "uz_outconv_fwd_xf: C=%d unsupported", C);
  UZ_REQUIRE(ldy % 8 == 0 && ldy >= C && N > 0 && HW > 0 && (long long)N * HW < (1LL << 31), "uz_outconv_fwd_xf: bad shape");
  const int ppb = 256 / lanes_per_pixel(C / 8);
  const int grid = grid_for(((long long)N * HW + ppb - 1) / ppb, 1);
  hipStream_t s = (hipStream_t)stream;
  UZ_KOUT_SWITCH(Kout, hipLaunchKernelGGL((outconv_fwd_kernel<bf16_t, KOUT, true>), dim3(grid), dim3(256), 0, s, (const bf16_t*)y, ldy, N, HW, C, w, b, out_nchw, scale, shift))
  UZ_LAUNCH_CHECK("uz_outconv_fwd_xf");
  return UZ_OK;
}

static int outconv_bwd_grid(int dtype, int N, int HW, int C) {
  const int vec = dtype == UZ_BF16 ? 8 : 4;
  const int ppb = 256 / lanes_per_pixel(C / vec);
  long long g = ((long long)N * HW + (long long)ppb * 4 - 1) / ((long long)ppb * 4);
  if (g > UZ_NUM_CU * 4) g = UZ_NUM_CU * 4;
  if (g < 1) g = 1;
  return (int)g;
}

extern "C" long long uz_outconv_bwd_workspace_bytes(int dtype, int N, int HW, int C, int Kout) {
  UZ_REQUIRE(dtype == UZ_F32 || dtype == UZ_BF16, "uz_outconv_bwd_workspace_bytes: bad dtype");
  const int vec = dtype == UZ_BF16 ? 8 : 4;
  UZ_REQUIRE(N > 0 && HW > 0 && Kout >= 1 && Kout <= OUTCONV_MAXK && C % vec == 0 && C / vec <= 64,
             "uz_outconv_bwd_workspace_bytes: bad shape");
  return (long long)outconv_bwd_grid(dtype, N, HW, C) * Kout * (C + 1) * (long long)sizeof(float);
}

extern "C" int uz_outconv_bwd_rows(int dtype, int N, int HW, int C) {
  UZ_REQUIRE(dtype == UZ_F32 || dtype == UZ_BF16, "uz_outconv_bwd_rows: bad dtype");
  return outconv_bwd_grid(dtype, N, HW, C);
}

extern "C" int uz_outconv_bwd_bnred(int dtype, const void* x, int ldx, int N, int HW, int C, const float* w,
                                    int Kout, const float* g_nchw, void* dx, int lddx, float* dw, float* db,
                                    void* workspace, const void* bn_y, int ld_bny, const float* scale,
                                    const float* shift, const float* mean, const float* invstd, float* bn_partial,
                                    void* stream) {
  UZ_REQUIRE(dtype == UZ_BF16, "uz_outconv_bwd_bnred: bf16 only");
  UZ_REQUIRE(w && g_nchw && dw && db && workspace && bn_y && scale && shift && mean && invstd && bn_partial,
             "uz_outconv_bwd_bnred: null pointer");
  UZ_REQUIRE(Kout >= 1 && Kout <= OUTCONV_MAXK, "uz_outconv_bwd_bnred: Kout=%d", Kout);
  UZ_REQUIRE(C % 8 == 0 && C / 8 <= 64, "uz_outconv_bwd_bnred: C=%d unsupported", C);
  UZ_REQUIRE((x == nullptr || (ldx % 8 == 0 && ldx >= C)) && (dx == nullptr || (lddx % 8 == 0 && lddx >= C)) && ld_bny % 8 == 0 && ld_bny >= C && N > 0 &&
                 HW > 0 && (long long)N * HW < (1LL << 31), "uz_outconv_bwd_bnred: bad shape");
  const int g = outconv_bwd_grid(dtype, N, HW, C);
  float* part = static_cast<float*>(workspace);
  hipStream_t s = (hipStream_t)stream;
  if (x != nullptr) {
    UZ_KOUT_SWITCH(Kout, hipLaunchKernelGGL((outconv_bwd_kernel<bf16_t, KOUT, true>), dim3((unsigned)g), dim3(256), 0, s,
                                            (const bf16_t*)x, ldx, N, HW, C, w, g_nchw, (bf16_t*)dx, lddx, part,
                                            (const bf16_t*)bn_y, ld_bny, scale, shift, mean, invstd, bn_partial))
  } else {
    UZ_KOUT_SWITCH(Kout, hipLaunchKernelGGL((outconv_bwd_kernel<bf16_t, KOUT, true, true>), dim3((unsigned)g), dim3(256), 0, s,
                                            (const bf16_t*)nullptr, 0, N, HW, C, w, g_nchw, (bf16_t*)dx, lddx, part,
                                            (const bf16_t*)bn_y, ld_bny, scale, shift, mean, invstd, bn_partial))
  }
  UZ_LAUNCH_CHECK("uz_outconv_bwd_bnred");
  const int ne = Kout * (C + 1);
  hipLaunchKernelGGL(outconv_bwd_finalize_kernel, dim3(uz_cdiv(ne, 32)), dim3(1024), 0, s, part, g, Kout, C, dw, db);
  UZ_LAUNCH_CHECK("uz_outconv_bwd_bnred(finalize)");
  return UZ_OK;
}

extern "C" int uz_outconv_bwd(int dtype, const void* x, int ldx, int N, int HW, int C, const float* w,
                              int Kout, const float* g_nchw, void* dx, int lddx, float* dw, float* db,
                              void* workspace, void* stream) {
  UZ_REQUIRE(dtype == UZ_F32 || dtype == UZ_BF16, "uz_outconv_bwd: bad dtype");
  const int vec = dtype == UZ_BF16 ? 8 : 4;
  UZ_REQUIRE(x && w && g_nchw && dw && db && workspace, "uz_outconv_bwd: null pointer");
  UZ_REQUIRE(Kout >= 1 && Kout <= OUTCONV_MAXK, "uz_outconv_bwd: Kout=%d", Kout);
  UZ_REQUIRE(C % vec == 0 && C / vec <= 64, "uz_outconv_bwd: C=%d unsupported", C);
  UZ_REQUIRE(ldx % vec == 0 && ldx >= C && N > 0 && HW > 0 && (long long)N * HW < (1LL << 31),
             "uz_outconv_bwd: bad shape");
  if (dx) UZ_REQUIRE(lddx % vec == 0 && lddx >= C, "uz_outconv_bwd: bad lddx");
  const int g = outconv_bwd_grid(dtype, N, HW, C);
  float* part = static_cast<float*>(workspace);
  hipStream_t s = (hipStream_t)stream;
  if (dtype == UZ_BF16) {
    UZ_KOUT_SWITCH(Kout, hipLaunchKernelGGL((outconv_bwd_kernel<bf16_t, KOUT>), dim3((unsigned)g), dim3(256), 0, s, (const bf16_t*)x, ldx, N, HW, C, w, g_nchw, (bf16_t*)dx, lddx, part, (const bf16_t*)nullptr, 0, (const float*)nullptr, (const float*)nullptr, (const float*)nullptr, (const float*)nullptr, (float*)nullptr))
  } else {
    UZ_KOUT_SWITCH(Kout, hipLaunchKernelGGL((outconv_bwd_kernel<float, KOUT>), dim3((unsigned)g), dim3(256), 0, s, (const float*)x, ldx, N, HW, C, w, g_nchw, (float*)dx, lddx, part, (const float*)nullptr, 0, (const float*)nullptr, (const float*)nullptr, (const float*)nullptr, (const float*)nullptr, (float*)nullptr))
  }
  UZ_LAUNCH_CHECK("uz_outconv_bwd");
  const int ne = Kout * (C + 1);
  hipLaunchKernelGGL(outconv_bwd_finalize_kernel, dim3(uz_cdiv(ne, 32)), dim3(1024), 0, s, part, g, Kout, C, dw, db);
  UZ_LAUNCH_CHECK("uz_outconv_bwd(finalize)");
  return UZ_OK;
}

extern "C" int uz_colsum(int dtype, const void* x, int ld, int P, int C, float* out, void* stream) {
  UZ_REQUIRE(dtype == UZ_F32 || dtype == UZ_BF16, "uz_colsum: bad dtype");
  const int vec = dtype == UZ_BF16 ? 8 : 4;
  UZ_REQUIRE(x && out && P > 0 && C > 0 && C % vec == 0 && ld % vec == 0 && ld >= C, "uz_colsum: bad args");
  dim3 grid, block;
  reduce_shape(C / vec, P, &grid, &block);
  const size_t shm = (size_t)256 * vec * sizeof(float);
  hipStream_t s = (hipStream_t)stream;
  if (dtype == UZ_BF16)
    hipLaunchKernelGGL((colsum_kernel<bf16_t, false>), grid, block, shm, s, (const bf16_t*)x, ld, (long long)P, C, out);
  else
    hipLaunchKernelGGL((colsum_kernel<float, false>), grid, block, shm, s, (const float*)x, ld, (long long)P, C, out);
  UZ_LAUNCH_CHECK("uz_colsum");
  return UZ_OK;
}

extern "C" long long uz_colsum_workspace_bytes(int dtype, int P, int C) {
  UZ_REQUIRE(dtype == UZ_F32 || dtype == UZ_BF16, "uz_colsum_workspace_bytes: bad dtype");
  const int vec = dtype == UZ_BF16 ? 8 : 4;
  UZ_REQUIRE(P > 0 && C > 0 && C % vec == 0, "uz_colsum_workspace_bytes: bad shape");
  dim3 grid, block;
  reduce_shape(C / vec, P, &grid, &block);
  return (long long)grid.x * C * (long long)sizeof(float);
}

extern "C" int uz_colsum_ws(int dtype, const void* x, int ld, int P, int C, float* out, void* workspace,
                            void* stream) {
  UZ_REQUIRE(dtype == UZ_F32 || dtype == UZ_BF16, "uz_colsum_ws: bad dtype");
  const int vec = dtype == UZ_BF16 ? 8 : 4;
  UZ_REQUIRE(x && out && workspace && P > 0 && C > 0 && C % vec == 0 && ld % vec == 0 && ld >= C, "uz_colsum_ws: bad args");
  dim3 grid, block;
  reduce_shape(C / vec, P, &grid, &block);
  const size_t shm = (size_t)256 * vec * sizeof(float);
  hipStream_t s = (hipStream_t)stream;
  float* part = static_cast<float*>(workspace);
  if (dtype == UZ_BF16)
    hipLaunchKernelGGL((colsum_kernel<bf16_t, true>), grid, block, shm, s, (const bf16_t*)x, ld, (long long)P, C, part);
  else
    hipLaunchKernelGGL((colsum_kernel<float, true>), grid, block, shm, s, (const float*)x, ld, (long long)P, C, part);
  UZ_LAUNCH_CHECK("uz_colsum_ws");
  hipLaunchKernelGGL(colsum_finalize_kernel, dim3(uz_cdiv(C, 32)), dim3(1024), 0, s, part, (int)grid.x, C, out);
  UZ_LAUNCH_CHECK("uz_colsum_ws(finalize)");
  return UZ_OK;
}

extern "C" int uz_colstats_rows(int dtype, int P, int C) {
  UZ_REQUIRE(dtype == UZ_F32 || dtype == UZ_BF16, "uz_colstats_rows: bad dtype");
  const int vec = dtype == UZ_BF16 ? 8 : 4;
  UZ_REQUIRE(P > 0 && C > 0 && C % vec == 0, "uz_colstats_rows: bad shape");
  dim3 grid, block;
  reduce_shape(C / vec, P, &grid, &block, 4);
  return (int)grid.x;
}

extern "C" int uz_colstats(int dtype, const void* x, int ld, int P, int C, float* partial, void* stream) {
  UZ_REQUIRE(dtype == UZ_F32 || dtype == UZ_BF16, "uz_colstats: bad dtype");
  const int vec = dtype == UZ_BF16 ? 8 : 4;
  UZ_REQUIRE(x && partial && P > 0 && C > 0 && C % vec == 0 && ld % vec == 0 && ld >= C, "uz_colstats: bad args");
  dim3 grid, block;
  reduce_shape(C / vec, P, &grid, &block, 4);
  const size_t shm = (size_t)256 * 2 * vec * sizeof(float);
  hipStream_t s = (hipStream_t)stream;
  if (dtype == UZ_BF16)
    hipLaunchKernelGGL((colstats_kernel<bf16_t>), grid, block, shm, s, (const bf16_t*)x, ld, (long long)P, C, partial);
  else
    hipLaunchKernelGGL((colstats_kernel<float>), grid, block, shm, s, (const float*)x, ld, (long long)P, C, partial);
  UZ_LAUNCH_CHECK("uz_colstats");
  return UZ_OK;
}

extern "C" int uz_pack_weights(int dtype, int mode, const float* w, int Co, int Ci, int T, int Kpad,
                               void* dst, void* stream) {
  UZ_REQUIRE(dtype == UZ_F32 || dtype == UZ_BF16, "uz_pack_weights: bad dtype");
  UZ_REQUIRE(w && dst && Co > 0 && Ci > 0 && T > 0, "uz_pack_weights: bad args");
  UZ_REQUIRE(mode >= UZ_PACK_CONV_FWD && mode <= UZ_PACK_IM2COL, "uz_pack_weights: bad mode %d", mode);
  long long total = (long long)Co * Ci * T;
  if (mode == UZ_PACK_IM2COL) {
    UZ_REQUIRE(Kpad >= T * Ci, "uz_pack_weights: Kpad too small");
    total = (long long)Co * Kpad;
  }
  hipStream_t s = (hipStream_t)stream;
  const int grid = grid_for(total, 256);
  if (dtype == UZ_BF16)
    hipLaunchKernelGGL((pack_weights_kernel<bf16_t>), dim3(grid), dim3(256), 0, s, mode, w, Co, Ci, T, Kpad, (bf16_t*)dst, total);
  else
    hipLaunchKernelGGL((pack_weights_kernel<float>), dim3(grid), dim3(256), 0, s, mode, w, Co, Ci, T, Kpad, (float*)dst, total);
  UZ_LAUNCH_CHECK("uz_pack_weights");
  return UZ_OK;
}

template <typename T>
__global__ __launch_bounds__(256) void pack_conv3x3_tiled_kernel(const uz_pack3x3_item* __restrict__ items,
                                                                 int n, int total_tiles) {
  constexpr int TP = 32 * 33 + 4;
  __shared__ float tile[9 * TP];
  for (int gt = blockIdx.x; gt < total_tiles; gt += gridDim.x) {
    int lo = 0, hi = n - 1;
    while (lo < hi) {
      const int mid = (lo + hi + 1) >> 1;
      if (items[mid].tile_begin <= gt) lo = mid; else hi = mid - 1;
    }
    const uz_pack3x3_item it = items[lo];
    const int tl = gt - it.tile_begin;
    const int tiles_ci = it.Ci / 32;
    T* __restrict__ df = static_cast<T*>(it.dst_fwd);
    T* __restrict__ dd = static_cast<T*>(it.dst_dgrad);
    const int co0 = (tl / tiles_ci) * 32, ci0 = (tl % tiles_ci) * 32;
    __syncthreads();
    float stage[36];
#pragma unroll
    for (int i = 0; i < 36; ++i) {
      const int e = threadIdx.x + 256 * i;
      const int co_l = e / 288, r = e - co_l * 288;
      stage[i] = it.src[((size_t)(co0 + co_l) * it.Ci + ci0) * 9 + r];
    }
#pragma unroll
    for (int i = 0; i < 36; ++i) {
      const int e = threadIdx.x + 256 * i;
      const int co_l = e / 288, r = e - co_l * 288;
      const int ci_l = r / 9, tap = r - ci_l * 9;
      tile[tap * TP + co_l * 33 + ci_l] = stage[i];
    }
    __syncthreads();
    constexpr int VEC = ElemTraits<T>::VEC, PPR = 32 / VEC;
    for (int e = threadIdx.x; e < 9 * 32 * PPR; e += 256) {
      const int part = e % PPR, row = e / PPR;
      const int y = row & 31, tap = row >> 5;
      if (df != nullptr) {
        Vec16<T> v;
#pragma unroll
        for (int k = 0; k < VEC; ++k) v.v[k] = (T)tile[tap * TP + y * 33 + part * VEC + k];
        st16(df + (size_t)(co0 + y) * 9 * it.Ci + tap * it.Ci + ci0 + part * VEC, v);
      }
      if (dd != nullptr) {
        Vec16<T> v;
#pragma unroll
        for (int k = 0; k < VEC; ++k) v.v[k] = (T)tile[tap * TP + (part * VEC + k) * 33 + y];
        st16(dd + (size_t)(ci0 + y) * 9 * it.Co + (8 - tap) * it.Co + co0 + part * VEC, v);
      }
    }
  }
}

extern "C" int uz_pack_conv3x3_batched(int dtype, const uz_pack3x3_item* items_device, int n_items,
                                       int total_tiles, void* stream) {
  UZ_REQUIRE(dtype == UZ_F32 || dtype == UZ_BF16, "uz_pack_conv3x3_batched: bad dtype");
  UZ_REQUIRE(items_device && n_items > 0 && total_tiles > 0, "uz_pack_conv3x3_batched: bad args");
  const dim3 grid(total_tiles < 4096 ? total_tiles : 4096);
  hipStream_t s = (hipStream_t)stream;
  if (dtype == UZ_BF16)
    hipLaunchKernelGGL((pack_conv3x3_tiled_kernel<bf16_t>), grid, dim3(256), 0, s, items_device, n_items, total_tiles);
  else
    hipLaunchKernelGGL((pack_conv3x3_tiled_kernel<float>), grid, dim3(256), 0, s, items_device, n_items, total_tiles);
  UZ_LAUNCH_CHECK("uz_pack_conv3x3_batched");
  return UZ_OK;
}

extern "C" int uz_pack_weights_batched(int dtype, const uz_pack_item* items_device, int n_items,
                                       long long total_elements, void* stream) {
  UZ_REQUIRE(dtype == UZ_F32 || dtype == UZ_BF16, "uz_pack_weights_batched: bad dtype");
  UZ_REQUIRE(items_device && n_items > 0 && total_elements > 0, "uz_pack_weights_batched: bad args");
  hipStream_t s = (hipStream_t)stream;
  UZ_REQUIRE(n_items <= 65535, "uz_pack_weights_batched: too many items");
  const dim3 grid(n_items <= 16 ? 512 : (n_items <= 40 ? 256 : 128), n_items);
  if (dtype == UZ_BF16)
    hipLaunchKernelGGL((pack_weights_batched_kernel<bf16_t>), grid, dim3(256), 0, s, items_device, n_items, total_elements);
  else
    hipLaunchKernelGGL((pack_weights_batched_kernel<float>), grid, dim3(256), 0, s, items_device, n_items, total_elements);
  UZ_LAUNCH_CHECK("uz_pack_weights_batched");
  return UZ_OK;
}

extern "C" int uz_im2col3x3_nchw(int dtype, const float* x_nchw, int N, int C, int H, int W, int Kpad,
                                 void* dst, void* stream) {
  UZ_REQUIRE(dtype == UZ_F32 || dtype == UZ_BF16, "uz_im2col3x3_nchw: bad dtype");
  UZ_REQUIRE(x_nchw && dst && N > 0 && C > 0 && H > 0 && W > 0 && Kpad >= 9 * C, "uz_im2col3x3_nchw: bad args");
  const int vec_ = dtype == UZ_BF16 ? 8 : 4;
  UZ_REQUIRE(Kpad % vec_ == 0, "uz_im2col3x3_nchw: Kpad must be a multiple of %d", vec_);
  hipStream_t s = (hipStream_t)stream;
  const long long npix = (long long)N * H * W;
  if (C <= 4 && Kpad <= 64) {
    const int grid = grid_for(npix, 256);
#define UZ_IM2COL_C(TT, CC) \
  hipLaunchKernelGGL((im2col3x3_smallc_kernel<TT, CC>), dim3(grid), dim3(256), 0, s, x_nchw, N, H, W, Kpad, (TT*)dst, npix)
    if (dtype == UZ_BF16) {
      if (C == 1) UZ_IM2COL_C(bf16_t, 1); else if (C == 2) UZ_IM2COL_C(bf16_t, 2);
      else if (C == 3) UZ_IM2COL_C(bf16_t, 3); else UZ_IM2COL_C(bf16_t, 4);
    } else {
      if (C == 1) UZ_IM2COL_C(float, 1); else if (C == 2) UZ_IM2COL_C(float, 2);
      else if (C == 3) UZ_IM2COL_C(float, 3); else UZ_IM2COL_C(float, 4);
    }
#undef UZ_IM2COL_C
  } else {
    const long long total = npix * (Kpad / vec_);
    const int grid = grid_for(total, 256);
    if (dtype == UZ_BF16)
      hipLaunchKernelGGL((im2col3x3_kernel<bf16_t>), dim3(grid), dim3(256), 0, s, x_nchw, N, C, H, W, Kpad, (bf16_t*)dst, total);
    else
      hipLaunchKernelGGL((im2col3x3_kernel<float>), dim3(grid), dim3(256), 0, s, x_nchw, N, C, H, W, Kpad, (float*)dst, total);
  }
  UZ_LAUNCH_CHECK("uz_im2col3x3_nchw");
  return UZ_OK;
}

#include <atomic>
static std::atomic<int> g_cu_reserve{0};
int uz_num_cu() { return UZ_NUM_CU_HW - g_cu_reserve.load(std::memory_order_relaxed); }
extern "C" int uz_set_cu_reserve(int n) {
  UZ_REQUIRE(n >= 0 && n <= UZ_NUM_CU_HW / 2, "uz_set_cu_reserve: %d not in 0 .. %d", n, UZ_NUM_CU_HW / 2);
  g_cu_reserve.store(n, std::memory_order_relaxed);
  return UZ_OK;
}
extern "C" int uz_get_cu_reserve(void) { return g_cu_reserve.load(std::memory_order_relaxed); }

static thread_local char g_err[512] = "";
void uz_set_error(const char* fmt, ...) {
  va_list ap;
  va_start(ap, fmt);
  vsnprintf(g_err, sizeof(g_err), fmt, ap);
  va_end(ap);
}
extern "C" const char* uz_last_error_string(void) { return g_err; }

static thread_local hipEvent_t g_prof_e0 = nullptr, g_prof_e1 = nullptr;
static thread_local int g_prof_launches = -1;
bool uz_prof_take(hipEvent_t* e0, hipEvent_t* e1) {
  if (g_prof_launches < 0) return false;
  *e0 = g_prof_launches == 0 ? g_prof_e0 : nullptr;
  *e1 = g_prof_e1;
  ++g_prof_launches;
  return true;
}
extern "C" int uz_profile_arm(void* start_event, void* stop_event) {
  UZ_REQUIRE(start_event && stop_event, "uz_profile_arm: null event");
  g_prof_e0 = (hipEvent_t)start_event;
  g_prof_e1 = (hipEvent_t)stop_event;
  g_prof_launches = 0;
  return UZ_OK;
}
extern "C" int uz_profile_disarm(void) {
  const int n = g_prof_launches;
  g_prof_launches = -1;
  return n < 0 ? 0 : n;
}
extern "C" int uz_abi_version(void) { return UZ_ABI_VERSION; }
extern "C" int uz_build_ablate(void) {
#ifdef UZ_ABLATE
  return 1;
#else
  return 0;
#endif
}

namespace {

constexpr int ADAMW_ROWS = 1024;

__global__ __launch_bounds__(256) void sqnorm_partial_kernel(const float* __restrict__ g, long long n,
                                                             double* __restrict__ partial) {
  __shared__ double red[256];
  double s = 0.0;
  const long long n4 = n >> 2;
  const float4* g4 = reinterpret_cast<const float4*>(g);
  for (long long i = (long long)blockIdx.x * blockDim.x + threadIdx.x; i < n4; i += (long long)gridDim.x * blockDim.x) {
    const float4 v = g4[i];
    s += (double)(v.x * v.x + v.y * v.y) + (double)(v.z * v.z + v.w * v.w);
  }
  if (blockIdx.x == 0 && threadIdx.x < (n & 3)) {
    const float v = g[(n4 << 2) + threadIdx.x];
    s += (double)v * v;
  }
  red[threadIdx.x] = s;
  __syncthreads();
  for (int st = 128; st > 0; st >>= 1) {
    if ((int)threadIdx.x < st) red[threadIdx.x] += red[threadIdx.x + st];
    __syncthreads();
  }
  if (threadIdx.x == 0) partial[blockIdx.x] = red[0];
}

__global__ __launch_bounds__(256) void adamw_prepare_kernel(const double* __restrict__ partial, int rows, float max_norm,
                                                            float beta1, float beta2, float* __restrict__ step,
                                                            float* __restrict__ scal) {
  __shared__ double red[256];
  double s = 0.0;
  for (int i = threadIdx.x; i < rows; i += 256) s += partial[i];
  red[threadIdx.x] = s;
  __syncthreads();
  for (int st = 128; st > 0; st >>= 1) {
    if ((int)threadIdx.x < st) red[threadIdx.x] += red[threadIdx.x + st];
    __syncthreads();
  }
  if (threadIdx.x == 0) {
    const float norm = (float)sqrt(red[0]);
    float coef = 1.f;
    if (max_norm > 0.f) {
      coef = max_norm / (norm + 1e-6f);
      if (coef > 1.f) coef = 1.f;
    }
    const float t = step[0] + 1.f;
    step[0] = t;
    scal[0] = coef;
    scal[1] = 1.f - powf(beta1, t);
    scal[2] = 1.f - powf(beta2, t);
    scal[3] = norm;
  }
}

__global__ __launch_bounds__(256) void adamw_apply_kernel(float* __restrict__ p, const float* __restrict__ g,
                                                          float* __restrict__ m, float* __restrict__ v, long long n,
                                                          float lr, float beta1, float beta2, float eps, float wd,
                                                          const float* __restrict__ scal) {
  const float coef = scal[0], bc1 = scal[1], bc2 = scal[2];
  const float step_size = lr / bc1, rs2 = rsqrtf(bc2), decay = 1.f - lr * wd;
  auto upd = [&](float& pv, float gv, float& mv, float& vv) {
    gv *= coef;
    pv *= decay;
    mv = beta1 * mv + (1.f - beta1) * gv;
    vv = beta2 * vv + (1.f - beta2) * gv * gv;
    pv -= step_size * mv / (sqrtf(vv) * rs2 + eps);
  };
  const long long n4 = n >> 2;
  for (long long i = (long long)blockIdx.x * blockDim.x + threadIdx.x; i < n4; i += (long long)gridDim.x * blockDim.x) {
    float4 pv = reinterpret_cast<float4*>(p)[i], mv = reinterpret_cast<float4*>(m)[i], vv = reinterpret_cast<float4*>(v)[i];
    const float4 gv = reinterpret_cast<const float4*>(g)[i];
    upd(pv.x, gv.x, mv.x, vv.x);
    upd(pv.y, gv.y, mv.y, vv.y);
    upd(pv.z, gv.z, mv.z, vv.z);
    upd(pv.w, gv.w, mv.w, vv.w);
    reinterpret_cast<float4*>(p)[i] = pv;
    reinterpret_cast<float4*>(m)[i] = mv;
    reinterpret_cast<float4*>(v)[i] = vv;
  }
  if (blockIdx.x == 0 && threadIdx.x < (n & 3)) {
    const long long i = (n4 << 2) + threadIdx.x;
    upd(p[i], g[i], m[i], v[i]);
  }
}

}

extern "C" long long uz_clip_adamw_workspace_bytes(void) { return (long long)ADAMW_ROWS * 8 + 64; }

extern "C" int uz_clip_adamw(float* p, const float* g, float* m, float* v, long long n, float lr, float beta1,
                             float beta2, float eps, float weight_decay, float max_norm, float* step,
                             void* workspace, void* stream) {
  UZ_REQUIRE(p && g && m && v && step && workspace && n > 0, "uz_clip_adamw: bad args");
  UZ_REQUIRE((((uintptr_t)p | (uintptr_t)g | (uintptr_t)m | (uintptr_t)v | (uintptr_t)workspace) & 15) == 0,
             "uz_clip_adamw: buffers must be 16-byte aligned");
  hipStream_t s = (hipStream_t)stream;
  double* partial = static_cast<double*>(workspace);
  float* scal = reinterpret_cast<float*>(partial + ADAMW_ROWS);
  long long blocks = (n / 4 + 255) / 256;
  int rows = (int)(blocks < ADAMW_ROWS ? (blocks < 1 ? 1 : blocks) : ADAMW_ROWS);
  hipLaunchKernelGGL(sqnorm_partial_kernel, dim3(rows), dim3(256), 0, s, g, n, partial);
  UZ_LAUNCH_CHECK("uz_clip_adamw(norm)");
  hipLaunchKernelGGL(adamw_prepare_kernel, dim3(1), dim3(256), 0, s, partial, rows, max_norm, beta1, beta2, step, scal);
  UZ_LAUNCH_CHECK("uz_clip_adamw(prepare)");
  const int grid = (int)(blocks < UZ_NUM_CU * 8 ? (blocks < 1 ? 1 : blocks) : UZ_NUM_CU * 8);
  hipLaunchKernelGGL(adamw_apply_kernel, dim3(grid), dim3(256), 0, s, p, g, m, v, n, lr, beta1, beta2, eps, weight_decay, scal);
  UZ_LAUNCH_CHECK("uz_clip_adamw(apply)");
  return UZ_OK;
}
```

### unet_zoo_amd/engine.py

```python
from __future__ import annotations

import math
from types import SimpleNamespace
from typing import Callable, Dict, List, Optional, Sequence, Tuple

import torch
import torch.nn as nn

from . import _lib as L
from . import ops
from .ops import Act


def _round_up(a: int, b: int) -> int:
    return (a + b - 1) // b * b


def _bias_of(m: nn.Module) -> Optional[torch.Tensor]:
    return m.bias.detach() if m.bias is not None else None


class PackCache:

    def __init__(self):
        self.entries: Dict[tuple, tuple] = {}
        self._table: Optional[torch.Tensor] = None
        self._total = 0
        self._n = 0
        self._table_dtype = None
        self._table3: Optional[torch.Tensor] = None
        self._n3 = 0
        self._tiles3 = 0

    def invalidate(self) -> None:
        self.entries.clear()
        self._table = None

    def repoint(self) -> None:
        self._table = None

    def get(self, p: nn.Parameter, mode: int, kpad: int, dtype: torch.dtype) -> torch.Tensor:
        key = (id(p), mode, kpad, dtype)
        e = self.entries.get(key)
        if e is None:
            if mode == L.PACK_VEC_REPEAT:
                assert p.dtype == torch.float32 and p.is_contiguous(), "PACK_VEC_REPEAT takes a contiguous fp32 vector"
                dst = p.detach().repeat(kpad).contiguous()
            else:
                dst = ops.pack_weights(p.detach(), mode, dtype, kpad)
            self.entries[key] = (p, mode, kpad, dtype, dst)
            self._table = None
            return dst
        return e[4]

    def refresh(self, dtype: torch.dtype) -> None:
        ents = [e for e in self.entries.values() if e[3] == dtype]
        if not ents:
            return
        if self._table is None or self._table_dtype != dtype:
            self._build_tables(ents, dtype)
        lib = L.load()
        if self._n3 > 0:
            L.check(lib.uz_pack_conv3x3_batched(L.dtype_code(dtype), self._table3.data_ptr(), self._n3,
                                                self._tiles3, L.stream_ptr()), "uz_pack_conv3x3_batched")
        if self._n > 0:
            L.check(lib.uz_pack_weights_batched(L.dtype_code(dtype), self._table.data_ptr(), self._n,
                                                self._total, L.stream_ptr()), "uz_pack_weights_batched")

    def _build_tables(self, ents, dtype) -> None:
        dev = ents[0][4].device
        tiled = {}
        generic = []
        for (p, mode, kpad, _, dst) in ents:
            ok = (mode in (L.PACK_CONV_FWD, L.PACK_CONV_DGRAD) and p.dim() == 4 and tuple(p.shape[2:]) == (3, 3)
                  and p.shape[0] % 32 == 0 and p.shape[1] % 32 == 0)
            if ok:
                it = tiled.setdefault(id(p), [p, None, None])
                it[1 if mode == L.PACK_CONV_FWD else 2] = dst
            else:
                generic.append((p, mode, kpad, dst))
        arr3 = (L.Pack3x3Item * max(len(tiled), 1))()
        tb = 0
        for i, (p, df, dd) in enumerate(tiled.values()):
            arr3[i] = L.Pack3x3Item(p.data_ptr(), df.data_ptr() if df is not None else None,
                                    dd.data_ptr() if dd is not None else None, p.shape[0], p.shape[1], tb, 0)
            tb += (p.shape[0] // 32) * (p.shape[1] // 32)
        self._n3, self._tiles3 = len(tiled), tb
        self._table3 = torch.frombuffer(bytearray(bytes(arr3)), dtype=torch.uint8).to(dev)
        arr = (L.PackItem * max(len(generic), 1))()
        begin = 0
        for i, (p, mode, kpad, dst) in enumerate(generic):
            if mode == L.PACK_VEC_REPEAT:
                assert dst.dtype == torch.float32
                arr[i] = L.PackItem(p.data_ptr(), dst.data_ptr(), begin, mode, p.numel(), 1, kpad, 0, 0)
                begin += dst.numel()
                continue
            d0, d1 = p.shape[0], p.shape[1]
            T = p.numel() // (d0 * d1)
            co, ci = (d0, d1) if mode in (L.PACK_CONV_FWD, L.PACK_CONV_DGRAD, L.PACK_IM2COL) else (d1, d0)
            arr[i] = L.PackItem(p.data_ptr(), dst.data_ptr(), begin, mode, co, ci, T, kpad, 0)
            begin += dst.numel()
        self._table = torch.frombuffer(bytearray(bytes(arr)), dtype=torch.uint8).to(dev)
        self._total, self._n, self._table_dtype = begin, len(generic), dtype

class ImageInput:

    __slots__ = ("nchw", "kpad", "dtype", "_patches", "N", "H", "W")

    def __init__(self, nchw: torch.Tensor, kpad: int, dtype: torch.dtype):
        self.nchw, self.kpad, self.dtype, self._patches = nchw, kpad, dtype, None
        self.N, _, self.H, self.W = nchw.shape

    def patches(self) -> Act:
        if self._patches is None:
            self._patches = ops.im2col3x3_nchw(self.nchw, self.kpad, self.dtype)
        return self._patches


class Engine:
    direct_first_conv = True
    defer_linear_wgrads = True
    fuse_bn_reduce = True
    fuse_bn_reduce_convt = True
    fold_bn_apply = True
    fold_bn_apply_head = True
    fold_head_grad = True
    fold_first_bn_bwd = True
    fuse_bn_finalize = False
    FIN_FLAGS = 4096
    reverse_element_passes = True
    fold_bn_eval = False

    def __init__(self, dtype: torch.dtype, device: torch.device, training: bool, record: bool,
                 grad_sink: Optional[Callable[[nn.Parameter, torch.Tensor], None]] = None,
                 pack_cache: Optional[PackCache] = None, grads_in_place: bool = False,
                 fold_bn_eval: Optional[bool] = None):
        if fold_bn_eval is not None:
            self.fold_bn_eval = bool(fold_bn_eval)
        self.folded_layers = 0
        self.unfolded_layers = 0
        self.dtype = dtype
        self.device = device
        self.training = training
        self.record = record
        self.tape: List[Callable[[], None]] = []
        self.param_grads: Dict[nn.Parameter, torch.Tensor] = {}
        self.grad_sink = grad_sink
        self.bk = 64 if dtype == torch.bfloat16 else 32
        self._bn_channels = 0
        self._sums: Optional[torch.Tensor] = None
        self._sums_used = 0
        self._cache = pack_cache if pack_cache is not None else PackCache()
        self.grads_in_place = grads_in_place
        self._heads: List[Tuple[Callable[..., None], int]] = []
        self.grad_log: List[Tuple[int, nn.Parameter]] = []
        self._pending_colsums: List[Tuple[int, nn.Parameter, Act]] = []
        self._pending_rowsums: List[Tuple[int, Callable[[], None]]] = []
        self._pending_wgrads: List[Tuple[int, nn.Parameter, Act, Act]] = []
        self._rowsum_items: list = []
        self._cpb: Dict[nn.Module, dict] = {}
        self._bn_counters: List[torch.Tensor] = []
        self._cur_entry = -1
        self._fin_flags: Optional[torch.Tensor] = None
        self._fin_used = 0

    def _fin_flag(self) -> Optional[torch.Tensor]:
        if not self.fuse_bn_finalize:
            return None
        if self._fin_flags is None:
            self._fin_flags = torch.zeros(self.FIN_FLAGS, dtype=torch.int32, device=self.device)
        if self._fin_used >= self.FIN_FLAGS:
            return None
        self._fin_used += 1
        return self._fin_flags[self._fin_used - 1:self._fin_used]

    def new_act(self, N, H, W, C, needs_grad=True) -> Act:
        return ops.new_act(N, H, W, C, self.dtype, self.device, needs_grad)

    def new_cat(self, N, H, W, channels: Sequence[int]) -> Tuple[Act, List[Act]]:
        full = self.new_act(N, H, W, sum(channels))
        parts, o = [], 0
        for c in channels:
            parts.append(full.window(o, c))
            o += c
        full.parts = parts
        return full, parts

    def _dst(self, p: nn.Parameter) -> Optional[torch.Tensor]:
        if self.grads_in_place and p.grad is not None and p.grad.is_contiguous() and p.grad.dtype == torch.float32:
            return p.grad
        return None

    def _give_grad(self, p: nn.Parameter, g: Optional[torch.Tensor]) -> None:
        if not isinstance(p, nn.Parameter):
            return
        self.grad_log.append((self._cur_entry, p))
        if self.grads_in_place and p.grad is not None:
            if g is None:
                return
            if p in self.param_grads:
                if g.data_ptr() == p.grad.data_ptr():
                    raise RuntimeError("a parameter shared by two layers received its second gradient in place: "
                                       "shared parameters are not supported by the in-place (graphed) backward")
                p.grad.add_(g.reshape(p.grad.shape))
            elif g.data_ptr() != p.grad.data_ptr():
                p.grad.copy_(g.reshape(p.grad.shape))
            self.param_grads[p] = None
            if self.grad_sink is not None:
                self.grad_sink(p, p.grad)
            return
        if g is None:
            g = torch.zeros(p.shape, dtype=torch.float32, device=self.device)
        if p in self.param_grads:
            self.param_grads[p] = self.param_grads[p] + g
        else:
            self.param_grads[p] = g
        if self.grad_sink is not None:
            self.grad_sink(p, self.param_grads[p])

    def _bias_grad(self, p: nn.Parameter, g: Act) -> None:
        self._pending_colsums.append((self._cur_entry, p, g))

    def _linear_wgrad(self, p: nn.Parameter, g: Act, x: Act) -> None:
        if self.defer_linear_wgrads and self.dtype == torch.bfloat16:
            self._pending_wgrads.append((self._cur_entry, p, g, x))
        else:
            self._give_grad(p, ops.wgrad(g, x, tuple(p.shape), ntaps=1, out=self._dst(p)))

    def _after_rowsums(self, fn: Callable[[], None]) -> None:
        self._pending_rowsums.append((self._cur_entry, fn))

    def _flush_rowsums(self) -> None:
        if self._pending_rowsums:
            items, self._rowsum_items = self._rowsum_items, []
            after, self._pending_rowsums = self._pending_rowsums, []
            ops.sum_rows_f32_batched(items)
            cur = self._cur_entry
            for entry, fn in after:
                self._cur_entry = entry
                fn()
            self._cur_entry = cur

    def _flush_colsums(self) -> None:
        self._flush_rowsums()
        wpend, self._pending_wgrads = self._pending_wgrads, []
        if wpend:
            wouts = []
            for _, p, _, _ in wpend:
                dst = self._dst(p)
                wouts.append(dst if dst is not None else torch.empty(tuple(p.shape), dtype=torch.float32, device=self.device))
            ops.wgrad_multi([(g, x, o, 1, L.TAPS_CONV, 1) for (_, _, g, x), o in zip(wpend, wouts)])
            for (entry, p, _, _), o in zip(wpend, wouts):
                self._cur_entry = entry
                self._give_grad(p, o)
        pend, self._pending_colsums = self._pending_colsums, []
        if not pend:
            return
        outs = []
        for _, p, g in pend:
            dst = self._dst(p)
            outs.append(dst if dst is not None else torch.empty(g.C, dtype=torch.float32, device=self.device))
        ops.colsum_batched([(g, o) for (_, _, g), o in zip(pend, outs)])
        for (entry, p, _), o in zip(pend, outs):
            self._cur_entry = entry
            self._give_grad(p, o)

    def _pack(self, p: nn.Parameter, mode: int, kpad: int = 0) -> torch.Tensor:
        return self._cache.get(p, mode, kpad, self.dtype)

    def _bn_sums(self, C: int) -> torch.Tensor:
        if self._sums is None:
            self._sums = torch.empty(2 * self._bn_channels, dtype=torch.float64, device=self.device)
            self._sums_used = 0
        s = self._sums[self._sums_used:self._sums_used + 2 * C].view(2, C)
        self._sums_used += 2 * C
        return s

    def _sum_grads(self, a: Act, limit: int) -> List[Act]:
        gs = list(a.grads)
        while len(gs) > limit:
            x, y = gs.pop(), gs.pop()
            t = self.new_act(x.N, x.H, x.W, x.C)
            ops.add_acts(x, y, t)
            gs.append(t)
        return gs

    def input_im2col(self, x: torch.Tensor) -> "ImageInput":
        L.require_cuda(x)
        if x.dim() != 4:
            raise ValueError(f"expected a (N, C, H, W) input, got shape {tuple(x.shape)}")
        return ImageInput(x.contiguous().float(), _round_up(9 * x.shape[1], self.bk), self.dtype)

    def conv_bn_relu(self, x: Act, conv: nn.Conv2d, bn: nn.BatchNorm2d, *, out: Optional[Act] = None,
                     pool: bool = False, im2col: bool = False, upsample: bool = False,
                     residual: Optional[Act] = None, pool_ceil: bool = False, relu: bool = True,
                     stat_repeat: int = 1, sole_reader: bool = False,
                     defer_apply: Optional[nn.Conv2d] = None) -> Tuple[Act, Optional[Act]]:
        assert not (isinstance(x, Act) and x.lazy is not None) \
            or (sole_reader and not im2col and conv.kernel_size == (3, 3) and conv.dilation == (1, 1)), \
            "a lazy activation goes to the 3x3 convolution it was deferred for"
        xf = x.take_lazy() if isinstance(x, Act) else None
        N, H, W = (x.N, 2 * x.H, 2 * x.W) if upsample else (x.N, x.H, x.W)
        x, image, image_version, wp, ntaps, tmode, dil = self._lower_conv(x, conv, im2col, upsample)
        bare = not pool and residual is None and stat_repeat == 1
        if self.fold_bn_eval and not self.training and not self.record:
            act = self._conv_bn_relu_folded(x, conv, bn, out, image, wp, ntaps, dil, tmode, relu, N, H, W) \
                if (bare and xf is None) else None
            if act is not None:
                self.folded_layers += 1
                return act, None
            self.unfolded_layers += 1
        y = self.new_act(N, H, W, conv.out_channels)
        if image is not None:
            stats = ops.conv_first_fwd(image, conv.weight.detach(), _bias_of(conv), y, self.training)
        else:
            stats = ops.conv_igemm(x, wp, _bias_of(conv), y, ntaps=ntaps, dil=dil, taps_mode=tmode,
                                   want_stats=self.training, xform=xf)
        lazy = (defer_apply is not None and bare and relu and out is None
                and (self._defer_to_conv3x3(y, defer_apply) or self._defer_to_head(y, defer_apply)))
        fin = self._fin_flag() if (self.training and not lazy and stat_repeat == 1) else None
        vec = self._bn_vectors(bn, stats, y.P, stat_repeat) if fin is None else None
        if lazy:
            act, pooled = ops.Act(y.buf, y.off, y.C, N, H, W, True), None
            act.lazy = (vec[0], vec[1])
        else:
            act, pooled, vec = self._bn_relu_apply(y, bn, vec, stats, fin, out, pool, pool_ceil, residual, relu)
        if self.record and self.training and relu and pooled is None and residual is None and stat_repeat == 1:
            act.bn_src = (y, vec)
        if self.record:
            self._bn_channels += y.C
            lay = SimpleNamespace(x=x, conv=conv, bn=bn, y=y, vec=vec, act=act, pooled=pooled, residual=residual, relu=relu,
                                  pool_ceil=pool_ceil, frozen=not self.training, image=image, image_version=image_version,
                                  im2col=im2col, upsample=upsample, ntaps=ntaps, tmode=tmode, dil=dil, xf=xf,
                                  sole_reader=sole_reader)

            def bwd():
                r = self._conv_bn_relu_bwd_bn(lay)
                if r is not None:
                    self._conv_bn_relu_bwd_conv(lay, *r)

            self.tape.append(bwd)
        return act, pooled

    def _lower_conv(self, x, conv: nn.Conv2d, im2col: bool, upsample: bool):
        dil = conv.dilation[0]
        tmode = L.TAPS_CONV_UP2 if upsample else L.TAPS_CONV
        if im2col and isinstance(x, ImageInput):
            if (self.direct_first_conv and conv.kernel_size == (3, 3) and dil == 1 and conv.padding == (1, 1)
                    and conv.stride == (1, 1) and ops.conv_first_supported(self.dtype, x.nchw.shape[1], conv.out_channels)):
                return x, x.nchw, x.nchw._version, None, 1, tmode, dil
            x = x.patches()
        if im2col:
            return x, None, None, self._pack(conv.weight, L.PACK_IM2COL, x.C), 1, tmode, dil
        assert conv.kernel_size in ((3, 3), (1, 1)) and conv.in_channels == x.C
        ntaps = 9 if conv.kernel_size == (3, 3) else 1
        assert ntaps == 9 or not upsample
        return x, None, None, self._pack(conv.weight, L.PACK_CONV_FWD), ntaps, tmode, dil

    def _defer_to_conv3x3(self, y: Act, reader: nn.Conv2d) -> bool:
        c2 = reader.out_channels
        return (self.fold_bn_apply and self.dtype == torch.bfloat16 and reader.kernel_size == (3, 3)
                and reader.dilation == (1, 1) and reader.stride == (1, 1) and reader.in_channels == y.C
                and ops.conv_xform_supported(y, c2, c2)
                and ops.wgrad_xform_shapes_supported(y.N, y.H, y.W, c2, c2, y.C, y.ld, self.dtype))

    def _defer_to_head(self, y: Act, reader: nn.Conv2d) -> bool:
        return (self.fold_bn_apply and self.fold_bn_apply_head and reader.kernel_size == (1, 1) and reader.in_channels == y.C
                and (self.training or not self.record) and self.fuse_bn_reduce_convt
                and ops.outconv_xform_supported(y, reader.out_channels))

    def _bn_relu_apply(self, y: Act, bn, vec, stats, fin, out, pool: bool, pool_ceil: bool, residual, relu: bool):
        act = out if out is not None else self.new_act(y.N, y.H, y.W, y.C)
        ph, pw = ((y.H + 1) // 2, (y.W + 1) // 2) if pool_ceil else (y.H // 2, y.W // 2)
        pooled = self.new_act(y.N, ph, pw, y.C) if pool else None
        assert relu or residual is None
        if fin is not None:
            vec = ops.bn_relu_apply_fin(y, stats, y.P, bn.weight.detach(), bn.bias.detach(), bn.eps, self._momentum(bn),
                                        bn.running_mean, bn.running_var, fin, act, pooled, residual, pool_ceil, relu=relu)
        else:
            ops.bn_relu_apply(y, vec[0], vec[1], act, pooled, residual, pool_ceil, relu=relu,
                              reverse=self.reverse_element_passes)
        return act, pooled, vec

    def _conv_bn_relu_bwd_bn(self, s):
        y, bn, residual, act, pooled = s.y, s.bn, s.residual, s.act, s.pooled
        gs = self._sum_grads(act, 2)
        gp = self._sum_grads(pooled, 1)[0] if (pooled is not None and pooled.grads) else None
        g0, g1 = (gs + [None, None])[:2]
        if g0 is None and gp is None:
            return None
# ... 1529 lines not shown
```

### unet_zoo_amd/graph.py

```python
from __future__ import annotations

import os
from typing import Callable, List, Optional, Sequence, Tuple

import torch
import torch.nn as nn

from . import _lib as L
from .engine import Engine, PackCache

_DTYPES = {"bf16": torch.bfloat16, "bfloat16": torch.bfloat16, "fp32": torch.float32,
           "float32": torch.float32}
_default_dtype = _DTYPES[os.environ.get("UNET_ZOO_AMD_DTYPE", "bf16").lower()]


def set_default_dtype(dtype) -> None:
    global _default_dtype
    _default_dtype = _DTYPES[dtype.lower()] if isinstance(dtype, str) else dtype
    L.dtype_code(_default_dtype)


def get_default_dtype() -> torch.dtype:
    return _default_dtype


class _GraphFn(torch.autograd.Function):
    @staticmethod
    def forward(ctx, model: "HipModule", plist: List[nn.Parameter], record: bool, x: torch.Tensor,
                *params: torch.Tensor):
        model._pack_cache.refresh(model.run_dtype)
        eng = Engine(model.run_dtype, x.device, model.training, record, model._grad_sink,
                     model._pack_cache, model.grads_in_place)
        outs = model.emit(eng, x)
        eng.finish_forward()
        ctx.eng = eng if record else None
        ctx.plist = plist
        ctx.sink_done = model._grad_sink_done
        return tuple(outs)

    @staticmethod
    def backward(ctx, *grad_outputs):
        eng = ctx.eng
        if eng is None:
            raise RuntimeError("backward through a HipModule forward that ran without gradient recording")
        grads = eng.backward(grad_outputs)
        ctx.eng = None
        if ctx.sink_done is not None:
            ctx.sink_done(grads)
        out = []
        for i, p in enumerate(ctx.plist):
            out.append(grads.get(p) if ctx.needs_input_grad[4 + i] else None)
        grads.clear()
        return (None, None, None, None, *out)


class HipModule(nn.Module):

    def __init__(self):
        super().__init__()
        self.run_dtype: torch.dtype = get_default_dtype()
        self._grad_sink: Optional[Callable] = None
        self._grad_sink_done: Optional[Callable] = None
        self._pack_cache = PackCache()
        self.grads_in_place = False

    def _apply(self, fn, *args, **kwargs):
        self._pack_cache.invalidate()
        return super()._apply(fn, *args, **kwargs)

    def emit(self, eng: Engine, x: torch.Tensor) -> Sequence[torch.Tensor]:
        raise NotImplementedError

    def wrap_outputs(self, outs: Tuple[torch.Tensor, ...]):
        return outs[0]

    def forward(self, x: torch.Tensor):
        L.load()
        L.require_cuda(x)
        if x.requires_grad:
            raise NotImplementedError("gradients with respect to the input image are not produced")
        plist = list(self.parameters())
        record = torch.is_grad_enabled() and any(p.requires_grad for p in plist)
        outs = _GraphFn.apply(self, plist, record, x, *plist)
        return self.wrap_outputs(outs)


class PhasedStep:

    def __init__(self, model: HipModule, loss_fn: Callable):
        self.model = model
        self.loss_fn = loss_fn
        self.eng: Optional[Engine] = None
        self._gouts: Optional[Tuple[Optional[torch.Tensor], ...]] = None

    def forward(self, x: torch.Tensor, target: torch.Tensor) -> torch.Tensor:
        self.emit(x)
        return self.loss(target)

    def emit(self, x: torch.Tensor):
        m = self.model
        L.load()
        L.require_cuda(x)
        m._pack_cache.refresh(m.run_dtype)
        self.eng = Engine(m.run_dtype, x.device, m.training, True, None, m._pack_cache, True)
        with torch.no_grad():
            self._outs = tuple(m.emit(self.eng, x))
            self.eng.finish_forward()
        self.outputs = m.wrap_outputs(tuple(o.detach() for o in self._outs))
        return self.outputs

    def loss(self, target: torch.Tensor) -> torch.Tensor:
        direct = getattr(self.loss_fn, "direct", None)
        if direct is not None:
            res = direct(self.model.wrap_outputs(tuple(o.detach() for o in self._outs)), target)
            loss, gouts = res[0], res[-1]
            assert len(gouts) == len(self._outs)
            self._gouts = tuple(gouts)
            return loss.detach()
        leaves = tuple(o.detach().requires_grad_(True) for o in self._outs)
        with torch.enable_grad():
            loss = self.loss_fn(self.model.wrap_outputs(leaves), target)
            self._gouts = torch.autograd.grad(loss, leaves, allow_unused=True)
        return loss.detach()

    def set_output_grads(self, gouts: Sequence[Optional[torch.Tensor]]) -> None:
        self._gouts = tuple(gouts)

    @property
    def n_entries(self) -> int:
        return len(self.eng.tape)

    def backward(self, hi: int, lo: int, heads: bool) -> None:
        self.eng.backward_range(self._gouts if heads else None, hi, lo)

    def finish(self) -> None:
        self.eng.tape.clear()
        self.eng = None
        self._gouts = None
        self._outs = None

    def plan(self, fractions: Sequence[float] = (0.45, 0.85)):
        log = self.eng.grad_log
        n = self.n_entries
        last: dict = {}
        for pos, p in log:
            last[p] = pos if p not in last else min(last[p], pos)
        order = sorted(last.items(), key=lambda kv: -kv[1])
        total = sum(p.numel() for p, _ in order)
        cuts, groups, cur, acc, fi = [n], [], [], 0, 0
        fr = list(fractions)
        for idx, (p, pos) in enumerate(order):
            cur.append(p)
            acc += p.numel()
            nxt = order[idx + 1][1] if idx + 1 < len(order) else None
            if fi < len(fr) and acc >= fr[fi] * total and nxt is not None and nxt < pos:
                cuts.append(pos)
                groups.append(cur)
                cur = []
                while fi < len(fr) and acc >= fr[fi] * total:
                    fi += 1
        cuts.append(0)
        cur += [p for p in self.model.parameters() if p not in last and p.grad is not None]
        groups.append(cur)
        return cuts, groups
```

### unet_zoo_amd/optim.py

```python
from __future__ import annotations

from typing import Iterable, List, Sequence, Tuple

import torch
import torch.nn as nn

from . import _lib as L


class FlatClipAdamW:
    ALIGN = 64

    def __init__(self, params: Iterable[nn.Parameter], lr: float = 1e-3, betas: Tuple[float, float] = (0.9, 0.999),
                 eps: float = 1e-8, weight_decay: float = 1e-2, max_norm: float = 1.0):
        self.params: List[nn.Parameter] = list(params)
        assert self.params, "no parameters"
        dev = self.params[0].device
        L.require_cuda(*self.params)
        self.lr, self.betas, self.eps, self.weight_decay, self.max_norm = lr, betas, eps, weight_decay, max_norm
        A = self.ALIGN
        n = sum((p.numel() + A - 1) // A * A for p in self.params)
        self.n = n
        self.flat_p = torch.zeros(n, dtype=torch.float32, device=dev)
        self.flat_g = torch.zeros(n, dtype=torch.float32, device=dev)
        self.exp_avg = torch.zeros(n, dtype=torch.float32, device=dev)
        self.exp_avg_sq = torch.zeros(n, dtype=torch.float32, device=dev)
        self.step_count = torch.zeros(1, dtype=torch.float32, device=dev)
        off = 0
        self.spans = []
        for p in self.params:
            assert p.dtype == torch.float32
            k = p.numel()
            self.flat_p[off:off + k].copy_(p.detach().reshape(-1))
            p.data = self.flat_p[off:off + k].view_as(p)
            p.grad = self.flat_g[off:off + k].view_as(p)
            self.spans.append((off, off + (k + A - 1) // A * A))
            off += (k + A - 1) // A * A
        wsb = L.load().uz_clip_adamw_workspace_bytes()
        self._ws = torch.empty(wsb // 4, dtype=torch.float32, device=dev)

    def span_of(self, params: Sequence[nn.Parameter]) -> Tuple[int, int]:
        idx = [self.params.index(p) for p in params]
        assert idx == list(range(idx[0], idx[0] + len(idx))), "parameters are not consecutive in the flat order"
        return self.spans[idx[0]][0], self.spans[idx[-1]][1]

    def zero_grad(self) -> None:
        self.flat_g.zero_()

    @torch.no_grad()
    def step(self) -> None:
        L.check(L.load().uz_clip_adamw(self.flat_p.data_ptr(), self.flat_g.data_ptr(), self.exp_avg.data_ptr(),
                                       self.exp_avg_sq.data_ptr(), self.n, self.lr, self.betas[0], self.betas[1],
                                       self.eps, self.weight_decay, self.max_norm, self.step_count.data_ptr(),
                                       self._ws.data_ptr(), L.stream_ptr()), "uz_clip_adamw")

    def last_grad_norm(self) -> torch.Tensor:
        return self._ws[2048 + 3]
```

### unet_zoo_amd/step.py

```python
from __future__ import annotations

from typing import Callable, Dict, List, Optional, Sequence, Tuple, Union

import torch
import torch.distributed as dist
import torch.nn as nn

from .graph import PhasedStep
from .augment import GpuAugment
from .patches import PatchSampler
from .capture import CAPTURE_MODE, _check_capture, _new_graph, _unwrap, resolve_criterion, static_copy, unchanged
from .loss import MulticlassLoss, RegionLoss
from .optim import FlatClipAdamW


class _ShapeGraphs:
    __slots__ = ("x", "t", "mx", "mt", "aug", "src", "fwd", "phases", "gouts", "loss", "dice", "outputs", "pool", "ps", "tables")


class GraphedStep:
    def __init__(self, model: nn.Module, criterion: Union[str, RegionLoss, MulticlassLoss, Callable] = "bce_dice", *, lr: float = 1e-4,
                 betas: Tuple[float, float] = (0.9, 0.999), eps: float = 1e-8, weight_decay: float = 1e-5,
                 max_norm: float = 1.0, phases: int = 5, process_group=None, data_parallel: Optional[bool] = None,
                 cu_reserve: Optional[int] = None, comm: str = "overlap", comm_dtype: Optional[torch.dtype] = None,
                 augment: Optional[GpuAugment] = None, source: Optional[PatchSampler] = None):
        self.model = _unwrap(model)
        if cu_reserve is not None:
            from . import _lib
            _lib.set_cu_reserve(cu_reserve)
        fused, self._target_dtype = resolve_criterion(criterion)
        self._fused, self._fused_loss = fused, fused is not None
        self._loss_fn = (lambda out, t: fused[0](out, t)[0]) if fused is not None else criterion
        if augment is not None and not isinstance(augment, GpuAugment):
            raise TypeError(f"augment must be a unet_zoo_amd.GpuAugment, got {type(augment).__name__}")
        self.augment = augment
        if source is not None and not isinstance(source, PatchSampler):
            raise TypeError(f"source must be a unet_zoo_amd.PatchSampler, got {type(source).__name__}")
        if source is not None and source.out_mask is None:
            raise ValueError("source: the PatchSampler has no masks, a training step needs targets")
        if source is not None and source.out_mask.dtype != self._target_dtype:
            raise ValueError(f"source: the PatchSampler yields {source.out_mask.dtype} masks, the criterion takes {self._target_dtype} "
                             "targets (class indices go with MulticlassLoss, fp32 masks with every other criterion)")
        self.source = source
        self.lr, self.betas, self.eps, self.weight_decay, self.max_norm = lr, betas, eps, weight_decay, max_norm
        self.pg = process_group
        self.world = dist.get_world_size(process_group) if dist.is_initialized() else 1
        self.distributed = (self.world > 1) if data_parallel is None else bool(data_parallel)
        if self.distributed and not dist.is_initialized():
            raise RuntimeError("data_parallel=True needs an initialised torch.distributed process group")
        self._nccl = self.distributed and dist.get_backend(process_group) == "nccl"
        self.n_phases = max(1, int(phases)) if self.distributed else 1
        if comm not in ("overlap", "tail"):
            raise ValueError(f"comm must be 'overlap' or 'tail', got {comm!r}")
        self.comm = comm
        if comm_dtype not in (None, torch.float32, torch.bfloat16):
            raise ValueError(f"comm_dtype must be None, torch.float32 or torch.bfloat16, got {comm_dtype!r}")
        self.comm_dtype = torch.bfloat16 if comm_dtype == torch.bfloat16 else torch.float32
        self._comm_stream: Optional[torch.cuda.Stream] = None
        self._comm_bufs: Dict[tuple, tuple] = {}
        self.opt: Optional[FlatClipAdamW] = None
        self._g_opt: Optional[torch.cuda.CUDAGraph] = None
        self._cuts: Optional[List[int]] = None
        self._spans: List[Tuple[int, int]] = []
        self._graphs: Dict[tuple, _ShapeGraphs] = {}
        self._cur: Optional[_ShapeGraphs] = None
        self.loss: Optional[torch.Tensor] = None
        self.dice: Optional[torch.Tensor] = None
        self.outputs = None
        self.steps_done = 0

    def _dry_run(self, x: torch.Tensor, t: torch.Tensor):
        m = self.model
        for p in m.parameters():
            p.grad = None
        ps = PhasedStep(m, self._loss_fn)
        with unchanged(m, x.device):
            ps.forward(x, t)
            ps.backward(ps.n_entries, 0, True)
            K = self.n_phases
            fr = [0.85 * (i + 1) / (K - 1) for i in range(K - 1)] if K > 1 else []
            cuts, groups = ps.plan(fr)
            ps.finish()
        return cuts, groups

    def _setup(self, x: torch.Tensor, t: torch.Tensor) -> None:
        m = self.model
        if not m.training:
            raise RuntimeError("GraphedStep is the TRAINING step: call model.train() first "
                               "(evaluate with model.eval() and torch.no_grad() as the reference does)")
        cuts, groups = self._dry_run(x, t)
        ordered = [p for grp in groups for p in grp]
        if not ordered:
            raise RuntimeError("no parameter received a gradient")
        self.opt = FlatClipAdamW(ordered, lr=self.lr, betas=self.betas, eps=self.eps,
                                 weight_decay=self.weight_decay, max_norm=self.max_norm)
        m._pack_cache.repoint()
        m._pack_cache.refresh(m.run_dtype)
        A, off = FlatClipAdamW.ALIGN, 0
        self._spans = []
        for grp in groups:
            k = sum((p.numel() + A - 1) // A * A for p in grp)
            self._spans.append((off, off + k))
            off += k
        assert off == self.opt.n
        self._cuts = cuts
        if self.world > 1:
            self._broadcast(self.opt.flat_p)
            for b in m.buffers():
                self._broadcast(b)
        self._capture_opt()

    def _capture_opt(self) -> None:
        self._g_opt = _new_graph()
        with torch.cuda.graph(self._g_opt, capture_error_mode=CAPTURE_MODE):
            self.opt.step()
        _check_capture(self._g_opt, "optimizer graph")

    def set_lr(self, lr: float) -> None:
        self.lr = lr
        if self.opt is not None:
            self.opt.lr = lr
            torch.cuda.synchronize()
            self._capture_opt()

    def _capture(self, x: torch.Tensor, t: torch.Tensor, aug=None, src=None) -> _ShapeGraphs:
        g = _ShapeGraphs()
        g.x, g.t, g.mx, g.mt, g.aug, g.src = x, t, x, t, aug, src
        ps = PhasedStep(self.model, self._loss_fn)
        cuts = self._cuts
        g.phases, g.fwd, g.gouts, g.dice, pool = [], None, None, None, None
        torch.cuda.synchronize()
        if self._fused_loss:
            dice_box = []
            with_autograd, direct = self._fused

            def fused(out, tt):
                l, d = with_autograd(out, tt)
                dice_box.append(d)
                return l

            def fused_direct(out, tt):
                l, d, gouts = direct(out, tt)
                dice_box.append(d)
                return l, gouts
            fused.direct = fused_direct
            ps.loss_fn = fused
        else:
            g.fwd = _new_graph()
            with torch.cuda.graph(g.fwd, capture_error_mode=CAPTURE_MODE):
                if src is not None:
                    src.run()
                if aug is not None:
                    aug.run()
                ps.emit(g.mx)
            _check_capture(g.fwd, "forward graph")
            pool = g.fwd.pool()
            g.outputs = ps.outputs
            g.gouts = [torch.zeros_like(o) for o in ps._outs]
            ps.set_output_grads(g.gouts)
        for k in range(len(cuts) - 1):
            gk = _new_graph()
            with torch.cuda.graph(gk, pool=pool, capture_error_mode=CAPTURE_MODE):
                if k == 0 and self._fused_loss:
                    if src is not None:
                        src.run()
                    if aug is not None:
                        aug.run()
                    g.loss = ps.forward(g.mx, g.mt)
                    g.outputs = ps.outputs
                    g.dice = dice_box[-1].detach()
                ps.backward(cuts[k], cuts[k + 1], k == 0)
            _check_capture(gk, f"backward phase {k}")
            pool = gk.pool()
            g.phases.append(gk)
        g.ps = ps
        if self._fused_loss:
            ps.finish()
        else:
            ps.eng.tape.clear()
            ps.eng = None
        g.pool = pool
        c = self.model._pack_cache
        g.tables = (c._table, c._table3)
        return g

    def _broadcast(self, t: torch.Tensor) -> None:
        if self._nccl:
            dist.broadcast(t, src=0, group=self.pg)
        else:
            h = t.detach().cpu()
            dist.broadcast(h, src=0, group=self.pg)
            t.copy_(h)

    class _EventWait:

        def __init__(self, ev):
            self.ev = ev

        def wait(self):
            torch.cuda.current_stream().wait_event(self.ev)

    def _exchange_bf16(self, buf: torch.Tensor):
        n, W = buf.numel(), self.world
        shard = (n + W - 1) // W
        key = (buf.data_ptr(), n)
        if key not in self._comm_bufs:
            dev = buf.device
            self._comm_bufs[key] = (torch.zeros(W * shard, dtype=torch.bfloat16, device=dev),
                                    torch.empty(W * shard, dtype=torch.bfloat16, device=dev),
                                    torch.empty(shard, dtype=torch.bfloat16, device=dev))
        send, recv, mine = self._comm_bufs[key]
        if self._comm_stream is None:
            self._comm_stream = torch.cuda.Stream(device=buf.device)
        ready = torch.cuda.Event()
        ready.record()
        cs = self._comm_stream
        with torch.cuda.stream(cs):
            cs.wait_event(ready)
            send[:n].copy_(buf)
            dist.all_to_all_single(recv, send, group=self.pg)
            mine.copy_(recv.view(W, shard).float().sum(0).mul_(1.0 / W))
            dist.all_gather_into_tensor(send, mine, group=self.pg)
            buf.copy_(send[:n])
            done = torch.cuda.Event()
            done.record(cs)
        return GraphedStep._EventWait(done)

    def _all_reduce_avg(self, buf: torch.Tensor):
        if self.comm_dtype == torch.bfloat16:
            if self._nccl:
                return self._exchange_bf16(buf)
            h = buf.detach().to(torch.bfloat16).float().cpu()
            dist.all_reduce(h, op=dist.ReduceOp.SUM, group=self.pg)
            buf.copy_(h.mul_(1.0 / self.world).to(torch.bfloat16).float().to(buf.device))
            return None
        if self._nccl:
            return dist.all_reduce(buf, op=dist.ReduceOp.AVG, group=self.pg, async_op=True)
        h = buf.detach().cpu()
        dist.all_reduce(h, op=dist.ReduceOp.SUM, group=self.pg)
        buf.copy_(h.mul_(1.0 / self.world).to(buf.device))
        return None

    def forward_backward(self, x: Optional[torch.Tensor] = None, target: Optional[torch.Tensor] = None) -> torch.Tensor:
        if self.source is not None:
            if x is not None or target is not None:
                raise TypeError("this GraphedStep draws its batch from `source` (a PatchSampler): call it without arguments")
            key = ("source",)
        elif x is None or target is None:
            raise TypeError("GraphedStep takes a batch (x, target); only a step built with source= is called without one")
        else:
            key = (tuple(x.shape), tuple(target.shape))
        g = self._graphs.get(key)
        if g is None:
            dev = next(self.model.parameters()).device
            src = None
            if self.source is not None:
                src = self.source.bind()
                if src.out_image.device != dev:
                    raise ValueError(f"source: the PatchSampler's pool is on {src.out_image.device}, the model on {dev}")
                sx, st = src.run()
            else:
                sx, st = static_copy(x, dev), static_copy(target, dev, self._target_dtype)
            aug, mx, mt = None, sx, st
            if self.augment is not None:
                sx, st = sx.contiguous(), st.contiguous()
                aug = self.augment.bind(sx, st)
                mx, mt = aug.out_image, aug.out_mask
                mx.copy_(sx)
                mt.copy_(st)
            if self.opt is None:
                self._setup(mx, mt)
            g = self._graphs[key] = self._capture(mx, mt, aug, src)
            g.x, g.t = sx, st
        self._cur = g
        if g.src is None:
            if x.data_ptr() != g.x.data_ptr():
                g.x.copy_(x)
            if target.data_ptr() != g.t.data_ptr():
                g.t.copy_(target)
        if g.fwd is not None:
            g.fwd.replay()
            loss = g.ps.loss(g.mt)
            for dst, src in zip(g.gouts, g.ps._gouts):
                if src is None:
                    dst.zero_()
                else:
                    dst.copy_(src)
            self.loss = loss
        else:
            self.loss = g.loss
        self.dice, self.outputs = g.dice, g.outputs
        if self.distributed and self.comm == "tail":
            for gk in g.phases:
                gk.replay()
            w = self._all_reduce_avg(self.opt.flat_g[:self._spans[-1][1]])
            if w is not None:
                w.wait()
        elif self.distributed:
            works = []
            for gk, (a0, a1) in zip(g.phases, self._spans):
                gk.replay()
                works.append(self._all_reduce_avg(self.opt.flat_g[a0:a1]))
            for w in works:
                if w is not None:
                    w.wait()
        else:
            for gk in g.phases:
                gk.replay()
        return self.loss

    def autotune_comm(self, x: Optional[torch.Tensor] = None, target: Optional[torch.Tensor] = None, steps: int = 6) -> Dict[str, float]:
        if not self.distributed:
            return {}
        dev = next(self.model.parameters()).device
        out: Dict[str, float] = {}
        for mode in ("overlap", "tail"):
            self.comm = mode
            for _ in range(2):
                self(x, target)
            torch.cuda.synchronize(dev)
            if self.world > 1:
                dist.barrier(group=self.pg)
            e0, e1 = torch.cuda.Event(enable_timing=True), torch.cuda.Event(enable_timing=True)
            e0.record()
            for _ in range(steps):
                self(x, target)
            e1.record()
            torch.cuda.synchronize(dev)
            ms = torch.tensor([e0.elapsed_time(e1) / steps], dtype=torch.float64, device=dev if self._nccl else "cpu")
            if self.world > 1:
                dist.all_reduce(ms, op=dist.ReduceOp.MAX, group=self.pg)
            out[mode] = float(ms.item())
        self.comm = "tail" if out["tail"] < 0.99 * out["overlap"] else "overlap"
        return out

    def optimizer_step(self) -> None:
        self._g_opt.replay()
        self.steps_done += 1

    def __call__(self, x: Optional[torch.Tensor] = None, target: Optional[torch.Tensor] = None) -> torch.Tensor:
        loss = self.forward_backward(x, target)
        self.optimizer_step()
        return loss

    @property
    def grad_norm(self) -> torch.Tensor:
        return self.opt.last_grad_norm()

    @property
    def augmented(self) -> Optional[Tuple[torch.Tensor, torch.Tensor]]:
        g = self._cur
        return None if g is None or g.aug is None else (g.aug.out_image, g.aug.out_mask)

    @property
    def sampled(self) -> Optional[Tuple[torch.Tensor, torch.Tensor]]:
        g = self._cur
        return None if g is None or g.src is None else (g.src.out_image, g.src.out_mask)

    @property
    def coords(self) -> Optional[torch.Tensor]:
        g = self._cur
        return None if g is None or g.src is None else g.src.coords

    @property
    def flat_grad(self) -> torch.Tensor:
        return self.opt.flat_g[:self.opt.n]

    def describe(self) -> str:
        k = len(self._cuts) - 1 if self._cuts else self.n_phases
        opt = "hipGraph(clip+AdamW on flat buffers, 3 launches)"
        crit = "" if self._fused_loss else "hipGraph(fwd) + eager criterion + "
        head = [name for name, opt_in in (("PatchSampler", self.source), ("GpuAugment", self.augment)) if opt_in is not None]
        if head:
            crit = " + ".join(head) + " at the head of the first hipGraph + " + crit
        if not self.distributed:
            return f"{crit}hipGraph({'fwd+' if self._fused_loss else ''}bwd) + {opt}"
        mb = [round((a1 - a0) * 4 / 2 ** 20, 1) for a0, a1 in self._spans]
        if self.comm_dtype == torch.bfloat16:
            opt = "gradient exchange in bf16 (all-to-all, fp32 sum on arrival, all-gather) + " + opt
        if self.comm == "tail":
            return (f"{crit}{k} hipGraphs ({'fwd + ' if self._fused_loss else ''}backward phases), then ONE RCCL all-reduce of "
                    f"{round(sum(mb), 1)} MB + {opt}")
        return (f"{crit}{k} hipGraphs ({'fwd + ' if self._fused_loss else ''}backward phases) with async RCCL "
                f"all-reduce of {mb} MB overlapped with the next phase + {opt}")
```

Before: 2532 images/sec.

## Fuse AdamW update with packing of 3x3 conv weights into bf16 layouts

Adds a fused optimizer kernel that applies the clipped AdamW update to 3x3 conv weights tile by tile and writes the packed forward and dgrad bf16 weight copies directly from shared memory. The remaining parameters are updated by a range-table kernel. This removes the separate repacking pass, which re-read every fp32 weight at the start of the next step. It adds bookkeeping to keep the packed copies current when parameters change outside the optimizer. It also rewrites the AdamW arithmetic with explicit fma and contraction turned off.

```diff
diff --git a/include/unetzoo_hip.h b/include/unetzoo_hip.h
--- a/include/unetzoo_hip.h
+++ b/include/unetzoo_hip.h
@@ -330,6 +330,15 @@
 int uz_clip_adamw(float* p, const float* g, float* m, float* v, long long n, float lr, float beta1,
                   float beta2, float eps, float weight_decay, float max_norm, float* step, void* workspace,
                   void* stream);
+typedef struct uz_adamw_range {
+  long long begin, end;
+  int chunk_begin;
+  int pad_;
+} uz_adamw_range;
+int uz_clip_adamw_pack3x3(float* p, const float* g, float* m, float* v, long long n, float lr, float beta1,
+                          float beta2, float eps, float weight_decay, float max_norm, float* step, void* workspace,
+                          int dtype, const uz_pack3x3_item* items_device, int n_items, int total_tiles,
+                          const uz_adamw_range* ranges_device, int n_ranges, int total_chunks, void* stream);
 
 int uz_gelu_fwd(int dtype, const void* x, int ldx, void* y, int ldy, long long P, int C, void* stream);
 int uz_gelu_bwd(int dtype, const void* x, int ldx, const void* g, int ldg, void* dx, int lddx, long long P,
diff --git a/unet_zoo_amd/_lib.py b/unet_zoo_amd/_lib.py
--- a/unet_zoo_amd/_lib.py
+++ b/unet_zoo_amd/_lib.py
@@ -34,7 +34,7 @@
     "uz_winattn_fwd", "uz_winattn_bwd_rows", "uz_winattn_bwd",
     "uz_colsum_workspace_bytes", "uz_colsum_ws", "uz_colstats_rows", "uz_colstats", "uz_cpb_fwd", "uz_cpb_bwd",
     "uz_cpb_fwd_batched", "uz_cpb_bwd_batched_workspace_bytes", "uz_cpb_bwd_batched",
-    "uz_clip_adamw_workspace_bytes", "uz_clip_adamw",
+    "uz_clip_adamw_workspace_bytes", "uz_clip_adamw", "uz_clip_adamw_pack3x3",
     "uz_gelu_fwd", "uz_gelu_bwd", "uz_dwconv3x3", "uz_dwconv3x3_wgrad_rows", "uz_dwconv3x3_wgrad",
     "uz_space_to_depth", "uz_space_to_depth_crop", "uz_im2col_nchw", "uz_sra_fwd", "uz_sra_bwd_workspace_bytes", "uz_sra_bwd",
     "uz_bce_dice_workspace_bytes", "uz_bce_dice", "uz_colsum_batched_workspace_bytes", "uz_colsum_batched", "uz_sum_rows_f32_batched", "uz_conv_igemm_res", "uz_wgrad_multi_workspace_bytes", "uz_wgrad_multi", "uz_conv_igemm_res_ws",
@@ -137,6 +137,10 @@
 class Pack3x3Item(Structure):
     _fields_ = [("src", c_void_p), ("dst_fwd", c_void_p), ("dst_dgrad", c_void_p), ("Co", c_int), ("Ci", c_int),
                 ("tile_begin", c_int), ("pad_", c_int)]
+
+
+class AdamwRange(Structure):
+    _fields_ = [("begin", ctypes.c_longlong), ("end", ctypes.c_longlong), ("chunk_begin", c_int), ("pad_", c_int)]
 
 
 REGION_MAX_ITEMS = 64
@@ -312,6 +316,8 @@
     lib.uz_cpb_bwd_batched.argtypes = [vp, ip, vp, vp]
     lib.uz_clip_adamw_workspace_bytes.argtypes = []
     lib.uz_clip_adamw.argtypes = [vp, vp, vp, vp, ctypes.c_longlong, fp, fp, fp, fp, fp, fp, vp, vp, vp]
+    lib.uz_clip_adamw_pack3x3.argtypes = [vp, vp, vp, vp, ctypes.c_longlong, fp, fp, fp, fp, fp, fp, vp, vp,
+                                          ip, vp, ip, ip, vp, ip, ip, vp]
     lib.uz_wgrad_split.argtypes = [POINTER(WgradDesc)]
     lib.uz_wgrad_workspace_bytes.argtypes = [POINTER(WgradDesc)]
     lib.uz_wgrad.argtypes = [POINTER(WgradDesc), vp, vp, vp, vp, vp]
diff --git a/unet_zoo_amd/csrc/uz_eltwise.hip b/unet_zoo_amd/csrc/uz_eltwise.hip
--- a/unet_zoo_amd/csrc/uz_eltwise.hip
+++ b/unet_zoo_amd/csrc/uz_eltwise.hip
@@ -1829,10 +1829,35 @@
   return UZ_OK;
 }
 
+constexpr int PACK3_TP = 32 * 33 + 4;
+template <typename T>
+__device__ __forceinline__ void pack3x3_store_tile(const float* __restrict__ tile, const uz_pack3x3_item& it, int co0, int ci0) {
+  constexpr int TP = PACK3_TP;
+  T* __restrict__ df = static_cast<T*>(it.dst_fwd);
+  T* __restrict__ dd = static_cast<T*>(it.dst_dgrad);
+  constexpr int VEC = ElemTraits<T>::VEC, PPR = 32 / VEC;
+  for (int e = threadIdx.x; e < 9 * 32 * PPR; e += 256) {
+    const int part = e % PPR, row = e / PPR;
+    const int y = row & 31, tap = row >> 5;
+    if (df != nullptr) {
+      Vec16<T> v;
+#pragma unroll
+      for (int k = 0; k < VEC; ++k) v.v[k] = (T)tile[tap * TP + y * 33 + part * VEC + k];
+      st16(df + (size_t)(co0 + y) * 9 * it.Ci + tap * it.Ci + ci0 + part * VEC, v);
+    }
+    if (dd != nullptr) {
+      Vec16<T> v;
+#pragma unroll
+      for (int k = 0; k < VEC; ++k) v.v[k] = (T)tile[tap * TP + (part * VEC + k) * 33 + y];
+      st16(dd + (size_t)(ci0 + y) * 9 * it.Co + (8 - tap) * it.Co + co0 + part * VEC, v);
+    }
+  }
+}
+
 template <typename T>
 __global__ __launch_bounds__(256) void pack_conv3x3_tiled_kernel(const uz_pack3x3_item* __restrict__ items,
                                                                  int n, int total_tiles) {
-  constexpr int TP = 32 * 33 + 4;
+  constexpr int TP = PACK3_TP;
   __shared__ float tile[9 * TP];
   for (int gt = blockIdx.x; gt < total_tiles; gt += gridDim.x) {
     int lo = 0, hi = n - 1;
@@ -1843,8 +1868,6 @@
     const uz_pack3x3_item it = items[lo];
     const int tl = gt - it.tile_begin;
     const int tiles_ci = it.Ci / 32;
-    T* __restrict__ df = static_cast<T*>(it.dst_fwd);
-    T* __restrict__ dd = static_cast<T*>(it.dst_dgrad);
     const int co0 = (tl / tiles_ci) * 32, ci0 = (tl % tiles_ci) * 32;
     __syncthreads();
     float stage[36];
@@ -1862,23 +1885,7 @@
       tile[tap * TP + co_l * 33 + ci_l] = stage[i];
     }
     __syncthreads();
-    constexpr int VEC = ElemTraits<T>::VEC, PPR = 32 / VEC;
-    for (int e = threadIdx.x; e < 9 * 32 * PPR; e += 256) {
-      const int part = e % PPR, row = e / PPR;
-      const int y = row & 31, tap = row >> 5;
-      if (df != nullptr) {
-        Vec16<T> v;
-#pragma unroll
-        for (int k = 0; k < VEC; ++k) v.v[k] = (T)tile[tap * TP + y * 33 + part * VEC + k];
-        st16(df + (size_t)(co0 + y) * 9 * it.Ci + tap * it.Ci + ci0 + part * VEC, v);
-      }
-      if (dd != nullptr) {
-        Vec16<T> v;
-#pragma unroll
-        for (int k = 0; k < VEC; ++k) v.v[k] = (T)tile[tap * TP + (part * VEC + k) * 33 + y];
-        st16(dd + (size_t)(ci0 + y) * 9 * it.Co + (8 - tap) * it.Co + co0 + part * VEC, v);
-      }
-    }
+    pack3x3_store_tile<T>(tile, it, co0, ci0);
   }
 }
 
@@ -2047,35 +2054,149 @@
   }
 }
 
+struct AdamwCoef {
+  float coef, step_size, rs2, decay, beta1, beta2, omb1, omb2, eps;
+};
+__device__ __forceinline__ AdamwCoef adamw_coef(const float* __restrict__ scal, float lr, float beta1, float beta2, float eps,
+                                                float wd) {
+#pragma clang fp contract(off)
+  const float coef = scal[0], bc1 = scal[1], bc2 = scal[2];
+  return AdamwCoef{coef, lr / bc1, rsqrtf(bc2), __builtin_fmaf(-lr, wd, 1.f), beta1, beta2, 1.f - beta1, 1.f - beta2, eps};
+}
+__device__ __forceinline__ void adamw_update(const AdamwCoef& c, float& pv, float gv, float& mv, float& vv) {
+#pragma clang fp contract(off)
+  gv = gv * c.coef;
+  mv = __builtin_fmaf(c.beta1, mv, c.omb1 * gv);
+  vv = __builtin_fmaf(c.beta2, vv, (c.omb2 * gv) * gv);
+  const float q = (c.step_size * mv) / __builtin_fmaf(sqrtf(vv), c.rs2, c.eps);
+  pv = __builtin_fmaf(c.decay, pv, -q);
+}
+__device__ __forceinline__ void adamw_update4(const AdamwCoef& c, float4& pv, const float4& gv, float4& mv, float4& vv) {
+  adamw_update(c, pv.x, gv.x, mv.x, vv.x);
+  adamw_update(c, pv.y, gv.y, mv.y, vv.y);
+  adamw_update(c, pv.z, gv.z, mv.z, vv.z);
+  adamw_update(c, pv.w, gv.w, mv.w, vv.w);
+}
+
 __global__ __launch_bounds__(256) void adamw_apply_kernel(float* __restrict__ p, const float* __restrict__ g,
                                                           float* __restrict__ m, float* __restrict__ v, long long n,
                                                           float lr, float beta1, float beta2, float eps, float wd,
                                                           const float* __restrict__ scal) {
-  const float coef = scal[0], bc1 = scal[1], bc2 = scal[2];
-  const float step_size = lr / bc1, rs2 = rsqrtf(bc2), decay = 1.f - lr * wd;
-  auto upd = [&](float& pv, float gv, float& mv, float& vv) {
-    gv *= coef;
-    pv *= decay;
-    mv = beta1 * mv + (1.f - beta1) * gv;
-    vv = beta2 * vv + (1.f - beta2) * gv * gv;
-    pv -= step_size * mv / (sqrtf(vv) * rs2 + eps);
-  };
+  const AdamwCoef c = adamw_coef(scal, lr, beta1, beta2, eps, wd);
   const long long n4 = n >> 2;
   for (long long i = (long long)blockIdx.x * blockDim.x + threadIdx.x; i < n4; i += (long long)gridDim.x * blockDim.x) {
     float4 pv = reinterpret_cast<float4*>(p)[i], mv = reinterpret_cast<float4*>(m)[i], vv = reinterpret_cast<float4*>(v)[i];
     const float4 gv = reinterpret_cast<const float4*>(g)[i];
-    upd(pv.x, gv.x, mv.x, vv.x);
-    upd(pv.y, gv.y, mv.y, vv.y);
-    upd(pv.z, gv.z, mv.z, vv.z);
-    upd(pv.w, gv.w, mv.w, vv.w);
+    adamw_update4(c, pv, gv, mv, vv);
     reinterpret_cast<float4*>(p)[i] = pv;
     reinterpret_cast<float4*>(m)[i] = mv;
     reinterpret_cast<float4*>(v)[i] = vv;
   }
   if (blockIdx.x == 0 && threadIdx.x < (n & 3)) {
     const long long i = (n4 << 2) + threadIdx.x;
-    upd(p[i], g[i], m[i], v[i]);
-  }
+    adamw_update(c, p[i], g[i], m[i], v[i]);
+  }
+}
+
+template <typename T>
+__global__ __launch_bounds__(256, 3) void adamw_pack3x3_tiled_kernel(float* __restrict__ p, const float* __restrict__ g,
+                                                                  float* __restrict__ m, float* __restrict__ v, float lr,
+                                                                  float beta1, float beta2, float eps, float wd,
+                                                                  const float* __restrict__ scal,
+                                                                  const uz_pack3x3_item* __restrict__ items, int n,
+                                                                  int total_tiles) {
+  constexpr int TP = PACK3_TP;
+  __shared__ float tile[9 * TP];
+  const AdamwCoef c = adamw_coef(scal, lr, beta1, beta2, eps, wd);
+  for (int gt = blockIdx.x; gt < total_tiles; gt += gridDim.x) {
+    int lo = 0, hi = n - 1;
+    while (lo < hi) {
+      const int mid = (lo + hi + 1) >> 1;
+      if (items[mid].tile_begin <= gt) lo = mid; else hi = mid - 1;
+    }
+    const uz_pack3x3_item it = items[lo];
+    const int tl = gt - it.tile_begin;
+    const int tiles_ci = it.Ci / 32;
+    const int co0 = (tl / tiles_ci) * 32, ci0 = (tl % tiles_ci) * 32;
+    const size_t base = (size_t)(it.src - p) + ((size_t)co0 * it.Ci + ci0) * 9;
+    float* __restrict__ pt = p + base;
+    const float* __restrict__ gt_ = g + base;
+    float* __restrict__ mt = m + base;
+    float* __restrict__ vt = v + base;
+    const unsigned row = (unsigned)it.Ci * 9u;
+    __syncthreads();
+#pragma unroll
+    for (int rd = 0; rd < 3; ++rd) {
+      float4 pv[3], gv[3], mv[3], vv[3];
+#pragma unroll
+      for (int j = 0; j < 3; ++j) {
+        const unsigned f = threadIdx.x + 256u * (rd * 3 + j);
+        const unsigned co_l = f / 72u, q = f - co_l * 72u;
+        const unsigned o = co_l * row + q * 4u;
+        pv[j] = *reinterpret_cast<const float4*>(pt + o);
+        gv[j] = *reinterpret_cast<const float4*>(gt_ + o);
+        mv[j] = *reinterpret_cast<const float4*>(mt + o);
+        vv[j] = *reinterpret_cast<const float4*>(vt + o);
+      }
+#pragma unroll
+      for (int j = 0; j < 3; ++j) {
+        const unsigned f = threadIdx.x + 256u * (rd * 3 + j);
+        const unsigned co_l = f / 72u, q = f - co_l * 72u;
+        const unsigned o = co_l * row + q * 4u;
+        adamw_update4(c, pv[j], gv[j], mv[j], vv[j]);
+        *reinterpret_cast<float4*>(pt + o) = pv[j];
+        *reinterpret_cast<float4*>(mt + o) = mv[j];
+        *reinterpret_cast<float4*>(vt + o) = vv[j];
+        const float w[4] = {pv[j].x, pv[j].y, pv[j].z, pv[j].w};
+#pragma unroll
+        for (int k = 0; k < 4; ++k) {
+          const unsigned r = q * 4u + k;
+          const unsigned ci_l = r / 9u, tap = r - ci_l * 9u;
+          tile[tap * TP + co_l * 33u + ci_l] = w[k];
+        }
+      }
+    }
+    __syncthreads();
+    pack3x3_store_tile<T>(tile, it, co0, ci0);
+  }
+}
+
+__global__ __launch_bounds__(256) void adamw_apply_ranges_kernel(float* __restrict__ p, const float* __restrict__ g,
+                                                                 float* __restrict__ m, float* __restrict__ v, float lr,
+                                                                 float beta1, float beta2, float eps, float wd,
+                                                                 const float* __restrict__ scal,
+                                                                 const uz_adamw_range* __restrict__ ranges, int n,
+                                                                 int total_chunks) {
+  const AdamwCoef c = adamw_coef(scal, lr, beta1, beta2, eps, wd);
+  for (int ch = blockIdx.x; ch < total_chunks; ch += gridDim.x) {
+    int lo = 0, hi = n - 1;
+    while (lo < hi) {
+      const int mid = (lo + hi + 1) >> 1;
+      if (ranges[mid].chunk_begin <= ch) lo = mid; else hi = mid - 1;
+    }
+    const uz_adamw_range r = ranges[lo];
+    const long long e = r.begin + (long long)(ch - r.chunk_begin) * 1024 + threadIdx.x * 4;
+    if (e < r.end) {
+      const long long i = e >> 2;
+      float4 pv = reinterpret_cast<float4*>(p)[i], mv = reinterpret_cast<float4*>(m)[i], vv = reinterpret_cast<float4*>(v)[i];
+      const float4 gv = reinterpret_cast<const float4*>(g)[i];
+      adamw_update4(c, pv, gv, mv, vv);
+      reinterpret_cast<float4*>(p)[i] = pv;
+      reinterpret_cast<float4*>(m)[i] = mv;
+      reinterpret_cast<float4*>(v)[i] = vv;
+    }
+  }
+}
+
+int adamw_norm_prepare(const float* g, long long n, float beta1, float beta2, float max_norm, float* step, double* partial,
+                       float* scal, hipStream_t s) {
+  long long blocks = (n / 4 + 255) / 256;
+  int rows = (int)(blocks < ADAMW_ROWS ? (blocks < 1 ? 1 : blocks) : ADAMW_ROWS);
+  hipLaunchKernelGGL(sqnorm_partial_kernel, dim3(rows), dim3(256), 0, s, g, n, partial);
+  UZ_LAUNCH_CHECK("uz_clip_adamw(norm)");
+  hipLaunchKernelGGL(adamw_prepare_kernel, dim3(1), dim3(256), 0, s, partial, rows, max_norm, beta1, beta2, step, scal);
+  UZ_LAUNCH_CHECK("uz_clip_adamw(prepare)");
+  return UZ_OK;
 }
 
 }
@@ -2091,14 +2212,45 @@
   hipStream_t s = (hipStream_t)stream;
   double* partial = static_cast<double*>(workspace);
   float* scal = reinterpret_cast<float*>(partial + ADAMW_ROWS);
-  long long blocks = (n / 4 + 255) / 256;
-  int rows = (int)(blocks < ADAMW_ROWS ? (blocks < 1 ? 1 : blocks) : ADAMW_ROWS);
-  hipLaunchKernelGGL(sqnorm_partial_kernel, dim3(rows), dim3(256), 0, s, g, n, partial);
-  UZ_LAUNCH_CHECK("uz_clip_adamw(norm)");
-  hipLaunchKernelGGL(adamw_prepare_kernel, dim3(1), dim3(256), 0, s, partial, rows, max_norm, beta1, beta2, step, scal);
-  UZ_LAUNCH_CHECK("uz_clip_adamw(prepare)");
+  const int rc = adamw_norm_prepare(g, n, beta1, beta2, max_norm, step, partial, scal, s);
+  if (rc != UZ_OK) return rc;
+  const long long blocks = (n / 4 + 255) / 256;
   const int grid = (int)(blocks < UZ_NUM_CU * 8 ? (blocks < 1 ? 1 : blocks) : UZ_NUM_CU * 8);
   hipLaunchKernelGGL(adamw_apply_kernel, dim3(grid), dim3(256), 0, s, p, g, m, v, n, lr, beta1, beta2, eps, weight_decay, scal);
   UZ_LAUNCH_CHECK("uz_clip_adamw(apply)");
   return UZ_OK;
 }
+
+extern "C" int uz_clip_adamw_pack3x3(float* p, const float* g, float* m, float* v, long long n, float lr, float beta1,
+                                     float beta2, float eps, float weight_decay, float max_norm, float* step,
+                                     void* workspace, int dtype, const uz_pack3x3_item* items_device, int n_items,
+                                     int total_tiles, const uz_adamw_range* ranges_device, int n_ranges, int total_chunks,
+                                     void* stream) {
+  UZ_REQUIRE(p && g && m && v && step && workspace && n > 0, "uz_clip_adamw_pack3x3: bad args");
+  UZ_REQUIRE((((uintptr_t)p | (uintptr_t)g | (uintptr_t)m | (uintptr_t)v | (uintptr_t)workspace) & 15) == 0,
+             "uz_clip_adamw_pack3x3: buffers must be 16-byte aligned");
+  UZ_REQUIRE(dtype == UZ_F32 || dtype == UZ_BF16, "uz_clip_adamw_pack3x3: bad dtype");
+  UZ_REQUIRE(items_device && n_items > 0 && total_tiles > 0, "uz_clip_adamw_pack3x3: no 3x3 items (use uz_clip_adamw)");
+  UZ_REQUIRE(n_ranges >= 0 && (n_ranges == 0 ? total_chunks == 0 : (ranges_device && total_chunks > 0)),
+             "uz_clip_adamw_pack3x3: bad range table");
+  hipStream_t s = (hipStream_t)stream;
+  double* partial = static_cast<double*>(workspace);
+  float* scal = reinterpret_cast<float*>(partial + ADAMW_ROWS);
+  const int rc = adamw_norm_prepare(g, n, beta1, beta2, max_norm, step, partial, scal, s);
+  if (rc != UZ_OK) return rc;
+  const dim3 grid(total_tiles < 4096 ? total_tiles : 4096);
+  if (dtype == UZ_BF16)
+    hipLaunchKernelGGL((adamw_pack3x3_tiled_kernel<bf16_t>), grid, dim3(256), 0, s, p, g, m, v, lr, beta1, beta2, eps,
+                       weight_decay, scal, items_device, n_items, total_tiles);
+  else
+    hipLaunchKernelGGL((adamw_pack3x3_tiled_kernel<float>), grid, dim3(256), 0, s, p, g, m, v, lr, beta1, beta2, eps,
+                       weight_decay, scal, items_device, n_items, total_tiles);
+  UZ_LAUNCH_CHECK("uz_clip_adamw_pack3x3(tiled)");
+  if (n_ranges > 0) {
+    const int rgrid = total_chunks < UZ_NUM_CU * 8 ? total_chunks : UZ_NUM_CU * 8;
+    hipLaunchKernelGGL(adamw_apply_ranges_kernel, dim3(rgrid), dim3(256), 0, s, p, g, m, v, lr, beta1, beta2, eps, weight_decay,
+                       scal, ranges_device, n_ranges, total_chunks);
+    UZ_LAUNCH_CHECK("uz_clip_adamw_pack3x3(ranges)");
+  }
+  return UZ_OK;
+}
diff --git a/unet_zoo_amd/engine.py b/unet_zoo_amd/engine.py
--- a/unet_zoo_amd/engine.py
+++ b/unet_zoo_amd/engine.py
@@ -1,6 +1,7 @@
 from __future__ import annotations
 
 import math
+from contextlib import contextmanager
 from types import SimpleNamespace
 from typing import Callable, Dict, List, Optional, Sequence, Tuple
 
@@ -18,6 +19,10 @@
 
 def _bias_of(m: nn.Module) -> Optional[torch.Tensor]:
     return m.bias.detach() if m.bias is not None else None
+
+
+def tiled3x3_eligible(shape) -> bool:
+    return len(shape) == 4 and tuple(shape[2:]) == (3, 3) and shape[0] % 32 == 0 and shape[1] % 32 == 0
 
 
 class PackCache:
@@ -31,13 +36,39 @@
         self._table3: Optional[torch.Tensor] = None
         self._n3 = 0
         self._tiles3 = 0
+        self._items3: list = []
+        self.copies3x3_current = False
+        self._trust3x3 = False
 
     def invalidate(self) -> None:
         self.entries.clear()
         self._table = None
+        self.copies3x3_current = False
 
     def repoint(self) -> None:
         self._table = None
+        self.copies3x3_current = False
+
+    def params_changed(self) -> None:
+        self.copies3x3_current = False
+
+    @contextmanager
+    def trusting_3x3(self):
+        self._trust3x3 = True
+        try:
+            yield
+        finally:
+            self._trust3x3 = False
+
+    def table3x3(self, dtype: torch.dtype) -> Optional[SimpleNamespace]:
+        ents = [e for e in self.entries.values() if e[3] == dtype]
+        if not ents:
+            return None
+        if self._table is None or self._table_dtype != dtype:
+            self._build_tables(ents, dtype)
+        if self._n3 == 0:
+            return None
+        return SimpleNamespace(table=self._table3, n=self._n3, tiles=self._tiles3, items=list(self._items3), dtype=dtype)
 
     def get(self, p: nn.Parameter, mode: int, kpad: int, dtype: torch.dtype) -> torch.Tensor:
         key = (id(p), mode, kpad, dtype)
@@ -60,7 +91,7 @@
         if self._table is None or self._table_dtype != dtype:
             self._build_tables(ents, dtype)
         lib = L.load()
-        if self._n3 > 0:
+        if self._n3 > 0 and not (self._trust3x3 and self.copies3x3_current):
             L.check(lib.uz_pack_conv3x3_batched(L.dtype_code(dtype), self._table3.data_ptr(), self._n3,
                                                 self._tiles3, L.stream_ptr()), "uz_pack_conv3x3_batched")
         if self._n > 0:
@@ -72,8 +103,7 @@
         tiled = {}
         generic = []
         for (p, mode, kpad, _, dst) in ents:
-            ok = (mode in (L.PACK_CONV_FWD, L.PACK_CONV_DGRAD) and p.dim() == 4 and tuple(p.shape[2:]) == (3, 3)
-                  and p.shape[0] % 32 == 0 and p.shape[1] % 32 == 0)
+            ok = mode in (L.PACK_CONV_FWD, L.PACK_CONV_DGRAD) and tiled3x3_eligible(p.shape)
             if ok:
                 it = tiled.setdefault(id(p), [p, None, None])
                 it[1 if mode == L.PACK_CONV_FWD else 2] = dst
@@ -86,6 +116,7 @@
                                     dd.data_ptr() if dd is not None else None, p.shape[0], p.shape[1], tb, 0)
             tb += (p.shape[0] // 32) * (p.shape[1] // 32)
         self._n3, self._tiles3 = len(tiled), tb
+        self._items3 = [tuple(it) for it in tiled.values()]
         self._table3 = torch.frombuffer(bytearray(bytes(arr3)), dtype=torch.uint8).to(dev)
         arr = (L.PackItem * max(len(generic), 1))()
         begin = 0
diff --git a/unet_zoo_amd/graph.py b/unet_zoo_amd/graph.py
--- a/unet_zoo_amd/graph.py
+++ b/unet_zoo_amd/graph.py
@@ -67,6 +67,12 @@
     def _apply(self, fn, *args, **kwargs):
         self._pack_cache.invalidate()
         return super()._apply(fn, *args, **kwargs)
+
+    def load_state_dict(self, *args, **kwargs):
+        try:
+            return super().load_state_dict(*args, **kwargs)
+        finally:
+            self._pack_cache.params_changed()
 
     def emit(self, eng: Engine, x: torch.Tensor) -> Sequence[torch.Tensor]:
         raise NotImplementedError
diff --git a/unet_zoo_amd/optim.py b/unet_zoo_amd/optim.py
--- a/unet_zoo_amd/optim.py
+++ b/unet_zoo_amd/optim.py
@@ -6,6 +6,30 @@
 import torch.nn as nn
 
 from . import _lib as L
+
+
+CHUNK = 1024
+
+
+def flat_spans(numels: Sequence[int], align: int) -> List[Tuple[int, int]]:
+    spans, off = [], 0
+    for k in numels:
+        padded = (k + align - 1) // align * align
+        spans.append((off, off + padded))
+        off += padded
+    return spans
+
+
+def complement_ranges(n: int, covered: Sequence[Tuple[int, int]]) -> List[Tuple[int, int]]:
+    out, at = [], 0
+    for b, e in sorted(covered):
+        assert at <= b < e <= n, "covered spans overlap or leave [0, n)"
+        if b > at:
+            out.append((at, b))
+        at = e
+    if at < n:
+        out.append((at, n))
+    return out
 
 
 class FlatClipAdamW:
@@ -26,16 +50,14 @@
         self.exp_avg = torch.zeros(n, dtype=torch.float32, device=dev)
         self.exp_avg_sq = torch.zeros(n, dtype=torch.float32, device=dev)
         self.step_count = torch.zeros(1, dtype=torch.float32, device=dev)
-        off = 0
-        self.spans = []
-        for p in self.params:
+        self.spans = flat_spans([p.numel() for p in self.params], A)
+        for p, (off, _) in zip(self.params, self.spans):
             assert p.dtype == torch.float32
             k = p.numel()
             self.flat_p[off:off + k].copy_(p.detach().reshape(-1))
             p.data = self.flat_p[off:off + k].view_as(p)
             p.grad = self.flat_g[off:off + k].view_as(p)
-            self.spans.append((off, off + (k + A - 1) // A * A))
-            off += (k + A - 1) // A * A
+        self._pack = None
         wsb = L.load().uz_clip_adamw_workspace_bytes()
         self._ws = torch.empty(wsb // 4, dtype=torch.float32, device=dev)
 
@@ -47,8 +69,44 @@
     def zero_grad(self) -> None:
         self.flat_g.zero_()
 
+    def prepare_pack(self, pack) -> bool:
+        self._pack = None
+        index = {id(p): i for i, p in enumerate(self.params)}
+        covered = []
+        for p, _, _ in pack.items:
+            i = index.get(id(p))
+            if i is None or p.data_ptr() != self.flat_p.data_ptr() + 4 * self.spans[i][0]:
+                return False
+            assert p.numel() % 4 == 0
+            covered.append((self.spans[i][0], self.spans[i][0] + p.numel()))
+        ranges = complement_ranges(self.n, covered)
+        arr = (L.AdamwRange * max(len(ranges), 1))()
+        chunks = 0
+        for i, (b, e) in enumerate(ranges):
+            assert b % 4 == 0 and e % 4 == 0
+            arr[i] = L.AdamwRange(b, e, chunks, 0)
+            chunks += (e - b + CHUNK - 1) // CHUNK
+        table = torch.frombuffer(bytearray(bytes(arr)), dtype=torch.uint8).to(self.flat_p.device)
+        self._pack = (pack, table, len(ranges), chunks)
+        return True
+
     @torch.no_grad()
-    def step(self) -> None:
+    def pack3x3_now(self) -> None:
+        pack = self._pack[0]
+        L.check(L.load().uz_pack_conv3x3_batched(L.dtype_code(pack.dtype), pack.table.data_ptr(), pack.n, pack.tiles,
+                                                 L.stream_ptr()), "uz_pack_conv3x3_batched")
+
+    @torch.no_grad()
+    def step(self, pack=None) -> None:
+        if pack is not None:
+            assert self._pack is not None and self._pack[0] is pack, "step(pack): prepare_pack(pack) comes first"
+            _, ranges, n_ranges, chunks = self._pack
+            L.check(L.load().uz_clip_adamw_pack3x3(
+                self.flat_p.data_ptr(), self.flat_g.data_ptr(), self.exp_avg.data_ptr(), self.exp_avg_sq.data_ptr(), self.n,
+                self.lr, self.betas[0], self.betas[1], self.eps, self.weight_decay, self.max_norm, self.step_count.data_ptr(),
+                self._ws.data_ptr(), L.dtype_code(pack.dtype), pack.table.data_ptr(), pack.n, pack.tiles,
+                ranges.data_ptr() if n_ranges else None, n_ranges, chunks, L.stream_ptr()), "uz_clip_adamw_pack3x3")
+            return
         L.check(L.load().uz_clip_adamw(self.flat_p.data_ptr(), self.flat_g.data_ptr(), self.exp_avg.data_ptr(),
                                        self.exp_avg_sq.data_ptr(), self.n, self.lr, self.betas[0], self.betas[1],
                                        self.eps, self.weight_decay, self.max_norm, self.step_count.data_ptr(),
diff --git a/unet_zoo_amd/step.py b/unet_zoo_amd/step.py
--- a/unet_zoo_amd/step.py
+++ b/unet_zoo_amd/step.py
@@ -1,5 +1,6 @@
 from __future__ import annotations
 
+from contextlib import nullcontext
 from typing import Callable, Dict, List, Optional, Sequence, Tuple, Union
 
 import torch
@@ -23,7 +24,7 @@
                  betas: Tuple[float, float] = (0.9, 0.999), eps: float = 1e-8, weight_decay: float = 1e-5,
                  max_norm: float = 1.0, phases: int = 5, process_group=None, data_parallel: Optional[bool] = None,
                  cu_reserve: Optional[int] = None, comm: str = "overlap", comm_dtype: Optional[torch.dtype] = None,
-                 augment: Optional[GpuAugment] = None, source: Optional[PatchSampler] = None):
+                 augment: Optional[GpuAugment] = None, source: Optional[PatchSampler] = None, fuse_pack: bool = True):
         self.model = _unwrap(model)
         if cu_reserve is not None:
             from . import _lib
@@ -58,6 +59,8 @@
         self.comm_dtype = torch.bfloat16 if comm_dtype == torch.bfloat16 else torch.float32
         self._comm_stream: Optional[torch.cuda.Stream] = None
         self._comm_bufs: Dict[tuple, tuple] = {}
+        self.fuse_pack = bool(fuse_pack)
+        self._pack = None
         self.opt: Optional[FlatClipAdamW] = None
         self._g_opt: Optional[torch.cuda.CUDAGraph] = None
         self._cuts: Optional[List[int]] = None
@@ -96,6 +99,11 @@
                                  weight_decay=self.weight_decay, max_norm=self.max_norm)
         m._pack_cache.repoint()
         m._pack_cache.refresh(m.run_dtype)
+        if self.fuse_pack:
+            pack = m._pack_cache.table3x3(m.run_dtype)
+            if pack is not None and self.opt.prepare_pack(pack):
+                self._pack = pack
+                m._pack_cache.copies3x3_current = True
         A, off = FlatClipAdamW.ALIGN, 0
         self._spans = []
         for grp in groups:
@@ -108,13 +116,23 @@
             self._broadcast(self.opt.flat_p)
             for b in m.buffers():
                 self._broadcast(b)
+            m._pack_cache.params_changed()
         self._capture_opt()
 
     def _capture_opt(self) -> None:
         self._g_opt = _new_graph()
         with torch.cuda.graph(self._g_opt, capture_error_mode=CAPTURE_MODE):
-            self.opt.step()
+            self.opt.step(self._pack)
         _check_capture(self._g_opt, "optimizer graph")
+
+    def params_changed(self) -> None:
+        self.model._pack_cache.params_changed()
+
+    def _ensure_copies(self) -> None:
+        c = self.model._pack_cache
+        if self._pack is not None and not c.copies3x3_current:
+            self.opt.pack3x3_now()
+            c.copies3x3_current = True
 
     def set_lr(self, lr: float) -> None:
         self.lr = lr
@@ -129,7 +147,15 @@
         ps = PhasedStep(self.model, self._loss_fn)
         cuts = self._cuts
         g.phases, g.fwd, g.gouts, g.dice, pool = [], None, None, None, None
+        self._ensure_copies()
         torch.cuda.synchronize()
+        with self.model._pack_cache.trusting_3x3() if self._pack is not None else nullcontext():
+            self._capture_graphs(g, ps, cuts, pool, aug, src)
+        c = self.model._pack_cache
+        g.tables = (c._table, c._table3)
+        return g
+
+    def _capture_graphs(self, g: _ShapeGraphs, ps: PhasedStep, cuts, pool, aug, src) -> None:
         if self._fused_loss:
             dice_box = []
             with_autograd, direct = self._fused
@@ -180,9 +206,6 @@
             ps.eng.tape.clear()
             ps.eng = None
         g.pool = pool
-        c = self.model._pack_cache
-        g.tables = (c._table, c._table3)
-        return g
 
     def _broadcast(self, t: torch.Tensor) -> None:
         if self._nccl:
@@ -273,6 +296,7 @@
             g = self._graphs[key] = self._capture(mx, mt, aug, src)
             g.x, g.t = sx, st
         self._cur = g
+        self._ensure_copies()
         if g.src is None:
             if x.data_ptr() != g.x.data_ptr():
                 g.x.copy_(x)
@@ -368,7 +392,8 @@
 
     def describe(self) -> str:
         k = len(self._cuts) - 1 if self._cuts else self.n_phases
-        opt = "hipGraph(clip+AdamW on flat buffers, 3 launches)"
+        opt = ("hipGraph(clip+AdamW on flat buffers writing the packed 3x3 weights, 4 launches)" if self._pack is not None
+               else "hipGraph(clip+AdamW on flat buffers, 3 launches)")
         crit = "" if self._fused_loss else "hipGraph(fwd) + eager criterion + "
         head = [name for name, opt_in in (("PatchSampler", self.source), ("GpuAugment", self.augment)) if opt_in is not None]
         if head:
```

Result: no change. 2537 images/sec, median of 6 (+0.2%).
